# Jittor/JNeRF

Hardware: NVIDIA H100
Metric: ngp_lego_train_rays_per_s (higher is better)
Workload: dtype f16

## Files before the change

### include/ngp_b200.h

```cpp
#ifndef NGP_B200_H
#define NGP_B200_H
#include <stdint.h>
#ifdef __cplusplus
extern "C" {
#endif

#define NGP_F32 0
#define NGP_F16 1
#define NGP_N_LEVELS 16
#define NGP_LEVEL_BYTES 32

const char* ngp_last_error(void);
int ngp_version(void);
int ngp_sm_count(void);
int ngp_debug_timeout_flag(void);

int ngp_hash_offsets(double aabb_scale, int n_levels, int base_resolution, int log2_hashmap_size,
                     uint32_t* offsets_out_host, double* per_level_scale_out);
int ngp_hash_level_table(void* stream, const uint32_t* offsets_host, int n_levels, uint32_t base_resolution,
                         float log2_per_level_scale, void* levels_dev);
int ngp_hash_level_table_primes(void* stream, const uint32_t* offsets_host, int n_levels, uint32_t base_resolution,
                                float log2_per_level_scale, void* levels_dev, uint32_t prime0, uint32_t prime1, uint32_t prime2);

int ngp_hash_fwd(void* stream, uint32_t n, const float* x, const void* grid, int dtype, const void* levels_dev, void* out);
int ngp_hash_bwd(void* stream, uint32_t n, const float* x, const void* dy, int dtype, const void* levels_dev,
                 void* grid_grad, uint64_t n_params);

int ngp_sh_fwd(void* stream, uint32_t n, const float* dirs, int dtype, void* out);

int ngp_mlp_fwd(void* stream, const void* weights, const void* input, void* inter, void* output,
                uint32_t n_hidden_matmuls, uint32_t n);
int ngp_mlp_bwd(void* stream, const void* weights, const void* input, const void* inter, const void* dY,
                void* dX, void* temps, float* dW, uint32_t n_hidden_matmuls, uint32_t n_out_valid, uint32_t n);
int ngp_mlp_bwd_dgrad(void* stream, const void* weights, const void* inter, const void* dY_feature_major, void* dX, void* temps,
                      uint32_t n_hidden_matmuls, uint32_t n);
int ngp_mlp_param_count(uint32_t n_hidden_matmuls);

int ngp_network_fwd(void* stream, uint32_t n_max, const uint32_t* n_dev, const float* coords, const void* grid,
                    const void* levels_dev, const void* w_density, const void* w_rgb, void* out, void* enc_save);
int ngp_network_bwd(void* stream, uint32_t n_max, const uint32_t* n_dev, const float* coords, const void* enc_save,
                    const void* levels_dev, const void* w_density, const void* w_rgb, const void* dout,
                    void* grid_grad, float* dw_density, float* dw_rgb);
int ngp_density_fwd(void* stream, uint32_t n, const float* pos, const void* grid, const void* levels_dev,
                    const void* w_density, void* sigma_out);

int ngp_mesh_workspace_bytes(uint32_t n, uint64_t n_verts, uint64_t n_tris, uint64_t* bytes_out);
int ngp_density_lattice(void* stream, uint32_t n, const void* grid, const void* levels_dev, const void* w_density, float* field_out);
int ngp_marching_cubes(void* stream, uint32_t n, const float* field, float iso, void* workspace, float* verts, uint64_t max_verts,
                       int32_t* tris, uint64_t max_tris, uint64_t* counts_host);
int ngp_mesh_largest_component(void* stream, uint64_t n_verts, uint64_t n_tris, const float* verts, const int32_t* tris, void* workspace,
                               float* verts_out, int32_t* tris_out, uint64_t* counts_host);
int ngp_mesh_vertex_normals(void* stream, uint64_t n_verts, uint64_t n_tris, const float* verts, const int32_t* tris, void* workspace,
                            float* normals);

uint64_t ngp_march_workspace_bytes(uint32_t n_rays);
int ngp_march(void* stream, uint32_t n_rays, float aabb_lo, float aabb_hi, uint32_t max_samples, const float* rays_o,
              const float* rays_d, const uint8_t* bitfield, float cone_angle, float near_distance, uint32_t cascades,
              int const_dt, uint64_t rng_state, uint64_t rng_inc, uint32_t* counters, uint32_t* ray_indices,
              uint32_t* numsteps, float* coords, void* workspace);
int ngp_compact(void* stream, uint32_t n_rays, uint32_t max_compacted, const float* coords_in, const uint32_t* numsteps_in,
                float* coords_out, uint32_t* numsteps_out, uint32_t* counters, int zero_fill);

int ngp_composite_fwd(void* stream, uint32_t n_rays, const void* net_out, int dtype, const float* coords,
                      const uint32_t* numsteps_in, const uint32_t* numsteps_compacted, const float* bg, uint32_t cascades,
                      float* rgb_out);
int ngp_composite_bwd(void* stream, uint32_t n_rays, uint32_t n_elements, const void* net_out, int dtype, const float* coords,
                      const uint32_t* numsteps_compacted, const float* loss_grad, const float* rgb_ray,
                      const float* density_grid_mean, uint32_t cascades, void* dnet_out);
int ngp_composite_infer(void* stream, uint32_t n_rays, const void* net_out, int dtype, const float* coords,
                        const uint32_t* numsteps, uint32_t cascades, float* rgb_out, float* alpha_out);
int ngp_composite_loss_bwd(void* stream, uint32_t n_rays, uint32_t n_elements, const void* net_out, const float* coords,
                           const uint32_t* numsteps_in, const uint32_t* numsteps_compacted, const float* bg,
                           const float* target, float huber_delta, const float* density_grid_mean, uint32_t cascades,
                           float* rgb_out, float* loss_out, void* dnet_out, float reg_scale);

int ngp_render_workspace_bytes(uint32_t n_rays, uint32_t capacity, uint64_t* layout_out);
int ngp_render_init(void* stream, uint32_t n_rays, uint32_t capacity, void* workspace, float aabb_lo, float aabb_hi, const float* rays_o,
                    const float* rays_d, float cone_angle, float near_distance, uint32_t cascades, int const_dt, uint64_t rng_state,
                    uint64_t rng_inc, uint32_t jitter_tile, float* rgb_out, float* alpha_out, uint32_t* n_samples_out, uint32_t* n_alive_host);
int ngp_render_march_round(void* stream, uint32_t n_rays, uint32_t capacity, void* workspace, uint32_t n_alive, uint32_t k_steps, float aabb_lo,
                           float aabb_hi, const float* rays_o, const float* rays_d, const uint8_t* bitfield, float cone_angle, uint32_t cascades,
                           int const_dt);
int ngp_render_composite_round(void* stream, uint32_t n_rays, uint32_t capacity, void* workspace, uint32_t n_alive, uint32_t k_steps,
                               float min_transmittance, uint32_t cascades, float* rgb_out, float* alpha_out, uint32_t* n_samples_out,
                               uint32_t* n_alive_host);

int ngp_grid_mark_untrained(void* stream, uint32_t n_elements, float* grid, uint32_t n_images, const float* focal_lengths,
                            const float* xforms, int res_x, int res_y);
int ngp_grid_generate_samples(void* stream, uint32_t n_elements, uint64_t rng_state, uint64_t rng_inc, const uint32_t* step_dev,
                              float aabb_lo, float aabb_hi, const float* grid_in, float* positions_out, uint32_t* indices_out,
                              uint32_t n_cascades, float thresh);
int ngp_grid_splat(void* stream, uint32_t n, const uint32_t* indices, const void* mlp_out, int dtype, float* grid_tmp);
int ngp_grid_ema(void* stream, uint32_t n_elements, float decay, float* grid, const float* grid_tmp);
int ngp_grid_update_bitfield(void* stream, const float* grid, float* mean_out, uint8_t* bitfield, uint32_t cascades);

int ngp_adam_ema(void* stream, uint64_t n, void* param, int param_dtype, void* grad, int grad_dtype, float grad_scale,
                 float* m, float* v, float* master, float lr, float beta1, float beta2, float eps, uint32_t step,
                 float ema_decay, int zero_grad);

int ngp_dp_exchange_step(void* stream, int world, int rank, uint64_t slice_len, uint32_t n_w, void* const* peer_table,
                         void* const* peer_table_grad, float* const* peer_w_grad, uint32_t* const* peer_flags, uint32_t epoch, float* m,
                         float* v, float* master, void* w_param, float* w_m, float* w_v, float* w_master, float grad_scale, float lr,
                         float beta1, float beta2, float eps, uint32_t step, float ema_decay);
int ngp_dp_exchange_wait(void* stream, int world, const uint32_t* my_flags, uint32_t epoch);
int ngp_ipc_export(const void* dev_ptr, uint8_t* handle64, uint64_t* offset);
int ngp_ipc_open(const uint8_t* handle64, uint64_t offset, void** dev_ptr);
int ngp_ipc_close(void* dev_ptr, uint64_t offset);

int ngp_raygen(void* stream, uint32_t n, const uint32_t* pix_index, uint32_t W, uint32_t H, const float* xforms,
               const float* focal, const float* principal, uint32_t* img_id_out, float* rays_o, float* rays_d);

int ngp_prepare_batch(void* stream, uint32_t n, const uint32_t* pix_index, uint32_t W, uint32_t H, const float* xforms,
                      const float* focal, const float* principal, const void* images_rgba, int image_is_u8, const float* bg,
                      uint32_t* img_id_out, float* rays_o, float* rays_d, float* target);

int ngp_blend_target(void* stream, uint32_t n, const float* rgba, const float* bg, float* target);

uint64_t ngp_step_state_bytes(void);
int ngp_step_state_set(void* stream, void* state_dev, uint64_t rng_state, uint64_t rng_inc, uint32_t pix_cursor, uint32_t adam_steps_done,
                       float lr, float beta1, float beta2, float eps, float ema_decay, float grad_scale);
int ngp_step_state_tick(void* stream, void* state_dev, uint32_t pix_advance, float lr, float beta1, float beta2, float eps,
                        float ema_decay, float grad_scale);
int ngp_prepare_batch_dev(void* stream, uint32_t n, const uint32_t* pix_list, const void* state_dev, uint32_t pix_offset, uint32_t W,
                          uint32_t H, const float* xforms, const float* focal, const float* principal, const void* images_rgba,
                          int image_is_u8, const float* bg, uint32_t* img_id_out, float* rays_o, float* rays_d, float* target);
int ngp_march_dev(void* stream, uint32_t n_rays, float aabb_lo, float aabb_hi, uint32_t max_samples, const float* rays_o,
                  const float* rays_d, const uint8_t* bitfield, float cone_angle, float near_distance, uint32_t cascades, int const_dt,
                  const void* state_dev, uint32_t ray_offset, uint32_t* counters, uint32_t* ray_indices, uint32_t* numsteps,
                  float* coords, void* workspace);
int ngp_adam_ema_dev(void* stream, uint64_t n, void* param, int param_dtype, void* grad, int grad_dtype, float* m, float* v,
                     float* master, const void* state_dev, int zero_grad);

void ngp_pcg32_seed(uint64_t initstate, uint64_t initseq, uint64_t* state_inc);
void ngp_pcg32_advance(uint64_t* state_inc, int64_t delta);

#ifdef __cplusplus
}
#endif
#endif
```

### jnerf_b200/csrc/fused_net.cu

```cuda
#include "mlp_tc.cuh"
#include <cstdlib>
#include <cstdio>
#include <mutex>
#include <vector>

int* ngp_err_flag();

namespace {
using namespace mlp;

constexpr int WD_W0 = 0, WD_WOUT = 64 * 32, WD_N = 64 * 32 + 16 * 64;
constexpr int WR_W0 = 0, WR_W1 = 64 * 32, WR_WOUT = 64 * 32 + 64 * 64, WR_N = 64 * 32 + 64 * 64 + 16 * 64;
constexpr int W_PART = WD_N + WR_N;

constexpr uint32_t G_ENC = 0, G_HD = 4, G_RIN = 12, G_H1 = 16, G_H2F = 4 , G_H2B = 24;
constexpr uint32_t G_ENC1 = 24;
struct SmemFwd {
    static constexpr uint32_t coords = 0;
    static constexpr uint32_t act = 8192;
    static constexpr uint32_t w0d = act + 28 * GB;
    static constexpr uint32_t woutd = w0d + 64 * 32 * 2;
    static constexpr uint32_t w0r = woutd + 16 * 64 * 2;
    static constexpr uint32_t w1r = w0r + 64 * 32 * 2;
    static constexpr uint32_t woutr = w1r + 64 * 64 * 2;
    static constexpr uint32_t levels = woutr + 16 * 64 * 2;
    static constexpr uint32_t total = levels + N_LEVELS * 32;
};
template <class S>
__device__ __forceinline__ void stage_all_weights(uint8_t* smem, const __half* wd, const __half* wr, uint32_t t) {
    stage_weights(smem + S::w0d, wd + WD_W0, 64, 32, t, 128);
    stage_weights(smem + S::woutd, wd + WD_WOUT, 16, 64, t, 128);
    if (wr) {
        stage_weights(smem + S::w0r, wr + WR_W0, 64, 32, t, 128);
        stage_weights(smem + S::w1r, wr + WR_W1, 64, 64, t, 128);
        stage_weights(smem + S::woutr, wr + WR_WOUT, 16, 64, t, 128);
    }
}

template <int STRIDE, int PTS>
__device__ __forceinline__ void gather_tile(const float* __restrict__ s_pos , const NgpLevel& lv,
                                            const __half2* __restrict__ g, uint8_t* act, uint32_t g_enc, uint32_t level, uint32_t sub,
                                            __half* __restrict__ enc_save, uint32_t tile_row0, uint32_t n_live) {
    uint32_t cgx = 0xffffffffu, cgy = 0, cgz = 0;
    __half2 v[8];
#pragma unroll
    for (int c = 0; c < 8; ++c) v[c] = __float2half2_rn(0.f);
#pragma unroll 1
    for (int k = 0; k < PTS; ++k) {
        const uint32_t p = PTS * sub + k;
        const HashCell hc = hash_cell(lv, s_pos[p * STRIDE], s_pos[p * STRIDE + 1], s_pos[p * STRIDE + 2]);
        if (hc.gx != cgx || hc.gy != cgy || hc.gz != cgz) {
            cgx = hc.gx; cgy = hc.gy; cgz = hc.gz;
            uint32_t idx[8];
            hash_cell_indices(lv, cgx, cgy, cgz, idx);
#pragma unroll
            for (int c = 0; c < 8; ++c) v[c] = __ldg(g + idx[c]);
        }
        float w[8];
        hash_cell_weights(hc, w);
        float a0 = 0.f, a1 = 0.f;
#pragma unroll
        for (int c = 0; c < 8; ++c) {
            const float2 f = __half22float2(v[c]);
            a0 = fmaf(w[c], f.x, a0);
            a1 = fmaf(w[c], f.y, a1);
        }
        const __half2 r = __floats2half2_rn(a0, a1);
        *reinterpret_cast<__half2*>(act + (size_t)(g_enc + (level >> 2)) * GB + p * 16 + (level & 3) * 4) = r;
        if (enc_save && tile_row0 + p < n_live)
            *reinterpret_cast<__half2*>(enc_save + (size_t)(tile_row0 + p) * 32 + 2 * level) = r;
    }
}

template <class S, uint32_t G_H2>
__device__ __forceinline__ void forward_chain(uint8_t* smem, uint32_t g_enc , uint32_t tw, bool density_only,
                                              uint32_t bar_id, uint16_t (&sig)[4]) {
    uint8_t* act = smem + S::act;
    const uint32_t smem_s = smem_u32(smem), act_s = smem_s + S::act;
    layer<64>([&](float (&d)[32], uint32_t m) { mma_fwd<32, 64>(d, act_s, g_enc, smem_s + S::w0d, m); },
              [&](const float (&d)[32], uint32_t m) { frag_to_slab<64, true>(d, act, G_HD, m, tw); });
    operands_ready(bar_id, 128);
    layer<16>([&](float (&d)[8], uint32_t m) { mma_fwd<64, 16>(d, act_s, G_HD, smem_s + S::woutd, m); },
              [&](const float (&d)[8], uint32_t m) {
                  sig[2 * m] = (uint16_t)(pack_half2(d[0], d[1]) & 0xFFFFu);
                  sig[2 * m + 1] = (uint16_t)(pack_half2(d[2], d[3]) & 0xFFFFu);
                  if (!density_only) frag_to_slab<16, false>(d, act, G_RIN, m, tw);
              });
    if (density_only) return;
    operands_ready(bar_id, 128);
    layer<64>([&](float (&d)[32], uint32_t m) { mma_fwd<32, 64>(d, act_s, G_RIN, smem_s + S::w0r, m); },
              [&](const float (&d)[32], uint32_t m) { frag_to_slab<64, true>(d, act, G_H1, m, tw); });
    operands_ready(bar_id, 128);
    layer<64>([&](float (&d)[32], uint32_t m) { mma_fwd<64, 64>(d, act_s, G_H1, smem_s + S::w1r, m); },
              [&](const float (&d)[32], uint32_t m) { frag_to_slab<64, true>(d, act, G_H2, m, tw); });
    operands_ready(bar_id, 128);
}
__device__ __forceinline__ void sh_to_slab(uint8_t* act, const float* s_coords, uint32_t t) {
    float sh[16];
    sh4(s_coords[t * 7 + 4], s_coords[t * 7 + 5], s_coords[t * 7 + 6], sh);
    uint32_t p[8];
#pragma unroll
    for (int i = 0; i < 8; ++i) p[i] = pack_half2(sh[2 * i], sh[2 * i + 1]);
    *reinterpret_cast<uint4*>(act + (G_RIN + 2) * GB + t * 16) = make_uint4(p[0], p[1], p[2], p[3]);
    *reinterpret_cast<uint4*>(act + (G_RIN + 3) * GB + t * 16) = make_uint4(p[4], p[5], p[6], p[7]);
}

constexpr int FWD_GW = 8;
constexpr int FWD_THREADS = 128 + 32 * FWD_GW;

__device__ __forceinline__ float lattice_coord(uint32_t r, uint32_t axis, uint32_t n) {
    const uint32_t idx = axis == 0 ? r / (n * n) : axis == 1 ? (r / n) % n : r % n;
    return __fdiv_rn((float)idx, (float)(n - 1));
}

template <bool DENSITY_ONLY, bool LATTICE = false>
__global__ void __launch_bounds__(FWD_THREADS, 2)
network_fwd_kernel(uint32_t n_max, const uint32_t* __restrict__ n_dev, const float* __restrict__ coords, const __half* __restrict__ grid,
                   const NgpLevel* __restrict__ levels, const __half* __restrict__ wd, const __half* __restrict__ wr,
                   __half* __restrict__ out, __half* __restrict__ enc_save, const __grid_constant__ NgpTensorMap enc_map, uint32_t enc_tma,
                   uint32_t lattice_n) {
    static_assert(DENSITY_ONLY || !LATTICE, "the lattice query is density only");
    extern __shared__ __align__(1024) uint8_t smem[];
    using S = SmemFwd;
    constexpr int CS = DENSITY_ONLY ? 3 : 7;
    const uint32_t t = threadIdx.x, warp = t >> 5;
    const bool is_chain = warp < 4;
    NgpLevel* s_lv = reinterpret_cast<NgpLevel*>(smem + S::levels);

    stage_weights(smem + S::w0d, wd + WD_W0, 64, 32, t, FWD_THREADS);
    stage_weights(smem + S::woutd, wd + WD_WOUT, 16, 64, t, FWD_THREADS);
    if (!DENSITY_ONLY) {
        stage_weights(smem + S::w0r, wr + WR_W0, 64, 32, t, FWD_THREADS);
        stage_weights(smem + S::w1r, wr + WR_W1, 64, 64, t, FWD_THREADS);
        stage_weights(smem + S::woutr, wr + WR_WOUT, 16, 64, t, FWD_THREADS);
    }
    if (t < N_LEVELS) s_lv[t] = levels[t];
    operands_ready(0, FWD_THREADS);
    const uint32_t n_live = n_dev ? min(*n_dev, n_max) : n_max;
    const uint32_t ntiles = (n_live + ROWS - 1) / ROWS;

    if (is_chain) {
        uint8_t* act = smem + S::act;
        const uint32_t smem_s = smem_u32(smem), r0 = frag_row(t);
        uint32_t it = 0;
        for (uint32_t tile = blockIdx.x; tile < ntiles; tile += gridDim.x, ++it) {
            const uint32_t buf = it & 1;
            const float* s_coords = reinterpret_cast<const float*>(smem + S::coords + buf * 3584);
            named_bar_sync(2 + buf, FWD_THREADS);
            if (!DENSITY_ONLY && enc_tma && warp == 0) {
                if (elect_one()) {
#pragma unroll
                    for (uint32_t g4 = 0; g4 < 4; ++g4)
                        tma_store_2d(&enc_map, 8 * g4, tile * ROWS, smem_s + S::act + ((buf ? G_ENC1 : G_ENC) + g4) * GB);
                    tma_store_commit();
                }
                __syncwarp();
            }
            if (!DENSITY_ONLY) sh_to_slab(act, s_coords, t);
            uint16_t sig[4];
            forward_chain<S, G_H2F>(smem, buf ? G_ENC1 : G_ENC, t, DENSITY_ONLY, 1, sig);
            if (!DENSITY_ONLY && enc_tma && warp == 0) {
                if (elect_one()) tma_store_wait_read();
                __syncwarp();
            }
            if (tile + 2 * gridDim.x < ntiles) named_bar_arrive(4 + buf, FWD_THREADS);
            if constexpr (DENSITY_ONLY) {
                if ((t & 3u) == 0) {
#pragma unroll
                    for (uint32_t i = 0; i < 4; ++i) {
                        const uint32_t row = tile * ROWS + 64 * (i >> 1) + r0 + 8 * (i & 1);
                        if (row >= n_live) continue;
                        if constexpr (LATTICE) reinterpret_cast<float*>(out)[row] = truncf(fmaxf(__half2float(__ushort_as_half(sig[i])), 0.f));
                        else reinterpret_cast<uint16_t*>(out)[row] = sig[i];
                    }
                }
            } else {
                layer<16>([&](float (&d)[8], uint32_t m) { mma_fwd<64, 16>(d, smem_s + S::act, G_H2F, smem_s + S::woutr, m); },
                          [&](const float (&d)[8], uint32_t m) {
#pragma unroll
                              for (uint32_t h = 0; h < 2; ++h) {
                                  const float c2 = __shfl_down_sync(0xffffffffu, d[2 * h], 1);
                                  const uint32_t row = tile * ROWS + 64 * m + r0 + 8 * h;
                                  if ((t & 3u) == 0 && row < n_live) {
                                      uint2 o;
                                      o.x = pack_half2(d[2 * h], d[2 * h + 1]);
                                      o.y = (pack_half2(c2, 0.f) & 0xFFFFu) | ((uint32_t)sig[2 * m + h] << 16);
                                      reinterpret_cast<uint2*>(out)[row] = o;
                                  }
                              }
                          });
            }
            named_bar_sync(1, 128);
        }
    } else {
        const uint32_t tg = t - 128, level = tg & 15, sub = tg >> 4;
        const NgpLevel lv = s_lv[level];
        const __half2* g = reinterpret_cast<const __half2*>(grid) + lv.offset;
        uint32_t it = 0;
        for (uint32_t tile = blockIdx.x; tile < ntiles; tile += gridDim.x, ++it) {
            const uint32_t buf = it & 1, row0 = tile * ROWS;
            float* s_coords = reinterpret_cast<float*>(smem + S::coords + buf * 3584);
            if (it >= 2) named_bar_sync(4 + buf, FWD_THREADS);
            for (uint32_t i = tg; i < ROWS * CS; i += 32 * FWD_GW) {
                if constexpr (LATTICE) s_coords[i] = (row0 + i / CS < n_live) ? lattice_coord(row0 + i / CS, i % CS, lattice_n) : 0.f;
                else s_coords[i] = (row0 + i / CS < n_live) ? __ldg(coords + (size_t)row0 * CS + i) : 0.f;
            }
            named_bar_sync(6, 32 * FWD_GW);
            gather_tile<CS, 64 / FWD_GW>(s_coords, lv, g, smem + S::act, buf ? G_ENC1 : G_ENC, level, sub, (DENSITY_ONLY || enc_tma) ? nullptr : enc_save, row0,
                                         n_live);
            fence_proxy_async_smem();
            named_bar_arrive(2 + buf, FWD_THREADS);
        }
    }
    if (!DENSITY_ONLY && enc_tma && warp == 0) {
        if (elect_one()) tma_store_wait_all();
        __syncwarp();
    }
}

constexpr uint32_t B3_G_GX = 32, B3_G_DY = 40, B3_G_DENC = 42, B3_GROUPS = 46;
constexpr uint32_t B3_EPI_THREADS = 256, B3_SCATTER_WARPS = 8, B3_THREADS = B3_EPI_THREADS + 32 * B3_SCATTER_WARPS;
constexpr uint32_t B3_RUNS = 12, B3_ITEMS = 16 * B3_RUNS, B3_RUN = (2 * 128 + B3_RUNS - 1) / B3_RUNS;
constexpr uint32_t B3_SCATTER_GROUPS = 32 * B3_SCATTER_WARPS / 4, B3_NI = B3_ITEMS / B3_SCATTER_GROUPS;
static_assert(B3_SCATTER_GROUPS % 16 == 0 && B3_ITEMS % B3_SCATTER_GROUPS == 0, "a lane group walks items of one level only, as many as every other group");
struct SmemBwd3 {
    static constexpr uint32_t coords = 0;
    static constexpr uint32_t tile0 = coords + 4 * 3584;
    static constexpr uint32_t tile_stride = B3_GROUPS * GB;
    static constexpr uint32_t w0d = tile0 + 2 * tile_stride;
    static constexpr uint32_t woutd = w0d + 64 * 32 * 2;
    static constexpr uint32_t w0r = woutd + 16 * 64 * 2;
    static constexpr uint32_t w1r = w0r + 64 * 32 * 2;
    static constexpr uint32_t woutr = w1r + 64 * 64 * 2;
    static constexpr uint32_t levels = woutr + 16 * 64 * 2;
    static constexpr uint32_t dsig = levels + N_LEVELS * 32;
    static constexpr uint32_t bar = dsig + 2 * ROWS * 2;
    static constexpr uint32_t total = bar + 16;
};
static_assert(SmemBwd3::total <= 227 * 1024, "backward CTA does not fit");
constexpr uint32_t B3_STAGE = 1, B3_FULL = 2, B3_EMPTY = 3;

constexpr float FX_SCALE = 4294967296.0f, FX_INV = 1.0f / 4294967296.0f;
__device__ __forceinline__ void red_add_fx(unsigned long long* p, float v) {
    const long long q = __float2ll_rn(fminf(fmaxf(v, -65504.f), 65504.f) * FX_SCALE);
    if (q) asm volatile("red.global.add.u64 [%0], %1;" ::"l"(__cvta_generic_to_global(p)), "l"((unsigned long long)q) : "memory");
}
__device__ __forceinline__ void red_add_entry_lane(unsigned long long* fx, uint32_t fx_live, __half2* gg, uint32_t idx, uint32_t f, float v) {
    if (idx < fx_live) {
        red_add_fx(fx + 2 * (size_t)idx + f, v);
    } else {
        const uint32_t lane = threadIdx.x & 31;
        const float o = __shfl_xor_sync(3u << (lane & 30), v, 1);
        if (!f) red_add_h2(gg + idx, v, o);
    }
}

template <uint32_t T>
__device__ __forceinline__ void bwd_chain(uint8_t* smem, uint32_t tid, uint32_t n_live, uint32_t npairs, const float* __restrict__ coords,
                                          const __half* __restrict__ enc_save, const __half* __restrict__ dout, float* __restrict__ w_part,
                                          float* __restrict__ dwd, float* __restrict__ dwr, int* __restrict__ err, uint32_t dbg, const NgpTensorMap* enc_map, uint32_t enc_tma) {
    using S = SmemBwd3;
    const uint32_t t = tid & 127, tq = (tid >> 5) & 3, r0 = frag_row(t);
    uint8_t* act = smem + S::tile0 + T * S::tile_stride;
    const uint32_t smem_s = smem_u32(smem), a0 = smem_s + S::tile0, a1 = a0 + S::tile_stride, a_s = T ? a1 : a0;
    __half* s_dsig = reinterpret_cast<__half*>(smem + S::dsig) + T * ROWS;
    uint64_t* bar_t = reinterpret_cast<uint64_t*>(smem + S::bar) + T;
    const bool wg = !(dbg & 4);
    float acc_woutr[8] = {}, acc_w1r[32] = {};
    float acc_w0r[16] = {}, acc_woutd[8] = {}, acc_w0d[16] = {};
    auto stage = [&]() { operands_ready(B3_STAGE, B3_EPI_THREADS); };
    float pf_c[7];
    uint4 pf_e[4];
    uint2 pf_d;
    auto prefetch = [&](uint32_t pair) {
        const uint32_t tile_ = 2 * pair + T, rr0 = tile_ * ROWS, r = rr0 + t;
        const bool ok = r < n_live;
#pragma unroll
        for (int j = 0; j < 7; ++j) {
            const uint32_t i = t + 128 * j;
            pf_c[j] = (rr0 + i / 7 < n_live) ? __ldg(coords + (size_t)rr0 * 7 + i) : 0.f;
        }
        if (!enc_tma) {
            const uint4* es = reinterpret_cast<const uint4*>(enc_save + (size_t)r * 32);
#pragma unroll
            for (int g = 0; g < 4; ++g) pf_e[g] = ok ? __ldg(es + g) : make_uint4(0, 0, 0, 0);
        }
        pf_d = ok ? __ldg(reinterpret_cast<const uint2*>(dout) + r) : make_uint2(0, 0);
    };
    if (blockIdx.x < npairs) prefetch(blockIdx.x);
    uint32_t it = 0, acc = 0;
    for (uint32_t pair = blockIdx.x; pair < npairs; pair += gridDim.x, ++it, acc = 1) {
        const uint32_t buf = it & 1;
        float* s_coords = reinterpret_cast<float*>(smem + S::coords + (2 * T + buf) * 3584);
        if (it >= 1) named_bar_sync(B3_STAGE, B3_EPI_THREADS);
#pragma unroll
        for (int j = 0; j < 7; ++j) s_coords[t + 128 * j] = pf_c[j];
        if (enc_tma) {
            if (tq == 0) {
                if (elect_one()) {
                    mbar_expect_tx(bar_t, ROWS * 64);
#pragma unroll
                    for (uint32_t g4 = 0; g4 < 4; ++g4)
                        tma_load_2d(smem_u32(act) + (G_ENC + g4) * GB, enc_map, 8 * g4, (2 * pair + T) * ROWS, bar_t);
                }
                __syncwarp();
            }
        } else {
#pragma unroll
            for (int g = 0; g < 4; ++g) *reinterpret_cast<uint4*>(act + (G_ENC + g) * GB + t * 16) = pf_e[g];
        }
        s_dsig[t] = __ushort_as_half((unsigned short)(pf_d.y >> 16));
        *reinterpret_cast<uint4*>(act + B3_G_DY * GB + t * 16) = make_uint4(pf_d.x, pf_d.y & 0xFFFFu, 0, 0);
        *reinterpret_cast<uint4*>(act + (B3_G_DY + 1) * GB + t * 16) = make_uint4(0, 0, 0, 0);
        if (pair + gridDim.x < npairs) prefetch(pair + gridDim.x);
        if (enc_tma) {
            if (!mbar_wait(bar_t, it & 1)) atomicExch(err, 4);
            if ((2 * pair + T) * ROWS + t >= n_live) {
#pragma unroll
                for (int g = 0; g < 4; ++g) *reinterpret_cast<uint4*>(act + (G_ENC + g) * GB + t * 16) = make_uint4(0, 0, 0, 0);
            }
        }
        named_bar_sync(4 + T, 128);
        sh_to_slab(act, s_coords, t);
        stage();
        layer<64>([&](float (&d)[32], uint32_t m) { mma_fwd<32, 64>(d, a_s, G_ENC, smem_s + S::w0d, m); },
                  [&](const float (&d)[32], uint32_t m) { frag_to_slab<64, true>(d, act, G_HD, m, t); });
        stage();
        layer<16>([&](float (&d)[8], uint32_t m) { mma_fwd<64, 16>(d, a_s, G_HD, smem_s + S::woutd, m); },
                  [&](const float (&d)[8], uint32_t m) { frag_to_slab<16, false>(d, act, G_RIN, m, t); });
        stage();
        layer<64>([&](float (&d)[32], uint32_t m) { mma_fwd<32, 64>(d, a_s, G_RIN, smem_s + S::w0r, m); },
                  [&](const float (&d)[32], uint32_t m) { frag_to_slab<64, true>(d, act, G_H1, m, t); });
        stage();
        layer<64>([&](float (&d)[32], uint32_t m) { mma_fwd<64, 64>(d, a_s, G_H1, smem_s + S::w1r, m); },
                  [&](const float (&d)[32], uint32_t m) { frag_to_slab<64, true>(d, act, G_H2B, m, t); });
        stage();
        if (T == 0 && wg) { wgmma_fence(); mma_wgrad<16>(acc_woutr, a0, G_H2B, a0, B3_G_DY, acc); mma_wgrad<16>(acc_woutr, a1, G_H2B, a1, B3_G_DY, 1); }
        layer<64>([&](float (&d)[32], uint32_t m) { mma_dgrad<16, 64>(d, a_s, B3_G_DY, smem_s + S::woutr, m); },
                  [&](const float (&d)[32], uint32_t m) { frag_dgrad_mask<64>(d, act, G_H2B, act, B3_G_GX, m, t); });
        stage();
        if (T == 0 && wg) { wgmma_fence(); mma_wgrad<64>(acc_w1r, a0, B3_G_GX, a0, G_H1, acc); mma_wgrad<64>(acc_w1r, a1, B3_G_GX, a1, G_H1, 1); }
        layer<64>([&](float (&d)[32], uint32_t m) { mma_dgrad<64, 64>(d, a_s, B3_G_GX, smem_s + S::w1r, m); },
                  [&](const float (&d)[32], uint32_t m) { frag_dgrad_mask<64>(d, act, G_H1, act, G_H2B, m, t); });
        stage();
        if (T == 1 && wg) { wgmma_fence(); mma_wgrad<32>(acc_w0r, a0, G_H2B, a0, G_RIN, acc); mma_wgrad<32>(acc_w0r, a1, G_H2B, a1, G_RIN, 1); }
        layer<16>([&](float (&d)[8], uint32_t m) { mma_dgrad<64, 16>(d, a_s, G_H2B, smem_s + S::w0r, m); },
                  [&](const float (&d)[8], uint32_t m) {
                      float v[8];
#pragma unroll
                      for (int i = 0; i < 8; ++i) v[i] = d[i];
                      if ((t & 3u) == 0) {
                          v[0] += __half2float(s_dsig[64 * m + r0]);
                          v[2] += __half2float(s_dsig[64 * m + r0 + 8]);
                      }
                      frag_to_slab<16, false>(v, act, B3_G_DY, m, t);
                  });
        stage();
        if (T == 1 && wg) { wgmma_fence(); mma_wgrad<16>(acc_woutd, a0, G_HD, a0, B3_G_DY, acc); mma_wgrad<16>(acc_woutd, a1, G_HD, a1, B3_G_DY, 1); }
        layer<64>([&](float (&d)[32], uint32_t m) { mma_dgrad<16, 64>(d, a_s, B3_G_DY, smem_s + S::woutd, m); },
                  [&](const float (&d)[32], uint32_t m) { frag_dgrad_mask<64>(d, act, G_HD, act, G_H1, m, t); });
        stage();
        if (T == 1 && wg) { wgmma_fence(); mma_wgrad<32>(acc_w0d, a0, G_H1, a0, G_ENC, acc); mma_wgrad<32>(acc_w0d, a1, G_H1, a1, G_ENC, 1); }
        if (it >= 1) named_bar_sync(B3_EMPTY, B3_EPI_THREADS + 32 * B3_SCATTER_WARPS);
        layer<32>([&](float (&d)[16], uint32_t m) { mma_dgrad<64, 32>(d, a_s, G_H1, smem_s + S::w0d, m); },
                  [&](const float (&d)[16], uint32_t m) { frag_to_slab<32, false>(d, act, B3_G_DENC, m, t); });
        named_bar_arrive(B3_FULL, B3_EPI_THREADS + 32 * B3_SCATTER_WARPS);
    }
    if (!w_part) {
        if (!it) return;
        if (T == 0) {
            frag_red_add<16>(acc_woutr, dwr + WR_WOUT, 1, 64, 64, 3, t);
            frag_red_add<64>(acc_w1r, dwr + WR_W1, 64, 1, 64, 64, t);
        } else {
            frag_red_add<32>(acc_w0r, dwr + WR_W0, 32, 1, 64, 32, t);
            frag_red_add<16>(acc_woutd, dwd + WD_WOUT, 1, 64, 64, 16, t);
            frag_red_add<32>(acc_w0d, dwd + WD_W0, 32, 1, 64, 32, t);
        }
        return;
    }
    dwd = w_part + (size_t)blockIdx.x * W_PART;
    dwr = dwd + WD_N;
    if (T == 0) {
        frag_store<16>(acc_woutr, dwr + WR_WOUT, 1, 64, 3, t);
        frag_store<64>(acc_w1r, dwr + WR_W1, 64, 1, 64, t);
    } else {
        frag_store<32>(acc_w0r, dwr + WR_W0, 32, 1, 32, t);
        frag_store<16>(acc_woutd, dwd + WD_WOUT, 1, 64, 16, t);
        frag_store<32>(acc_w0d, dwd + WD_W0, 32, 1, 32, t);
    }
}

__global__ void __launch_bounds__(B3_THREADS, 1)
network_bwd256_kernel(uint32_t n_max, const uint32_t* __restrict__ n_dev, const float* __restrict__ coords, const __half* __restrict__ enc_save,
                      const NgpLevel* __restrict__ levels, const __half* __restrict__ wd, const __half* __restrict__ wr,
                      const __half* __restrict__ dout, __half* __restrict__ grid_grad, float* __restrict__ dwd, float* __restrict__ dwr,
                      unsigned long long* __restrict__ grid_fx, uint32_t fx_entries, float* __restrict__ w_part,
                      int* __restrict__ err, uint32_t dbg, const __grid_constant__ NgpTensorMap enc_map, uint32_t enc_tma) {
    extern __shared__ __align__(1024) uint8_t smem[];
    using S = SmemBwd3;
    const uint32_t tid = threadIdx.x, warp = tid >> 5;
    uint64_t* bar_t = reinterpret_cast<uint64_t*>(smem + S::bar);
    NgpLevel* s_lv = reinterpret_cast<NgpLevel*>(smem + S::levels);

    stage_weights(smem + S::w0d, wd + WD_W0, 64, 32, tid, B3_THREADS);
    stage_weights(smem + S::woutd, wd + WD_WOUT, 16, 64, tid, B3_THREADS);
    stage_weights(smem + S::w0r, wr + WR_W0, 64, 32, tid, B3_THREADS);
    stage_weights(smem + S::w1r, wr + WR_W1, 64, 64, tid, B3_THREADS);
    stage_weights(smem + S::woutr, wr + WR_WOUT, 16, 64, tid, B3_THREADS);
    if (tid < N_LEVELS) s_lv[tid] = levels[tid];
    for (uint32_t i = tid; i < 2 * S::tile_stride / 16; i += B3_THREADS) *reinterpret_cast<uint4*>(smem + S::tile0 + i * 16) = make_uint4(0, 0, 0, 0);
    if (tid == 0) { mbar_init(bar_t, 1); mbar_init(bar_t + 1, 1); fence_mbar_init(); }
    operands_ready(0, B3_THREADS);
    const uint32_t n_live = n_dev ? min(*n_dev, n_max) : n_max;
    const uint32_t ntiles = (n_live + ROWS - 1) / ROWS, npairs = (ntiles + 1) / 2;

    if (warp < 4) {
        bwd_chain<0>(smem, tid, n_live, npairs, coords, enc_save, dout, w_part, dwd, dwr, err, dbg, &enc_map, enc_tma);
    } else if (warp < 8) {
        bwd_chain<1>(smem, tid, n_live, npairs, coords, enc_save, dout, w_part, dwd, dwr, err, dbg, &enc_map, enc_tma);
    } else {
        const uint32_t ts = tid - B3_EPI_THREADS, grp = ts >> 2, f = ts & 1, h = (ts >> 1) & 1;
        const uint32_t level = grp & 15;
        const NgpLevel lv = s_lv[level];
        unsigned long long* fx = grid_fx + 2 * (size_t)lv.offset;
        const uint32_t fx_live = fx_entries > lv.offset ? fx_entries - lv.offset : 0u;
        __half2* gg = reinterpret_cast<__half2*>(grid_grad) + lv.offset;
        uint32_t it = 0;
        for (uint32_t pair = blockIdx.x; pair < npairs; pair += gridDim.x, ++it) {
            const uint32_t buf = it & 1;
            named_bar_sync(B3_FULL, B3_EPI_THREADS + 32 * B3_SCATTER_WARPS);
            uint32_t cgx[B3_NI], cgy[B3_NI], cgz[B3_NI], idx[B3_NI][4];
            float acc[B3_NI][4];
            bool live[B3_NI], dirty[B3_NI];
#pragma unroll
            for (uint32_t i = 0; i < B3_NI; ++i) { cgx[i] = 0xffffffffu; cgy[i] = cgz[i] = 0; live[i] = !(dbg & 2); dirty[i] = false; }
#pragma unroll 1
            for (uint32_t k = 0; k < B3_RUN; ++k) {
                float2 df[B3_NI];
                HashCell hc[B3_NI];
#pragma unroll
                for (uint32_t i = 0; i < B3_NI; ++i) {
                    const uint32_t r = B3_RUN * ((grp + i * B3_SCATTER_GROUPS) >> 4) + k;
                    live[i] = live[i] && r < 2 * ROWS && 2 * pair * ROWS + r < n_live;
                    const uint32_t rc = min(r, 2 * ROWS - 1), T = rc >> 7, p = rc & 127;
                    const uint8_t* denc = smem + S::tile0 + T * S::tile_stride + B3_G_DENC * GB;
                    const float* s_coords = reinterpret_cast<const float*>(smem + S::coords + (2 * T + buf) * 3584);
                    df[i] = __half22float2(*reinterpret_cast<const __half2*>(denc + (size_t)(level >> 2) * GB + p * 16 + (level & 3) * 4));
                    hc[i] = hash_cell(lv, s_coords[p * 7], s_coords[p * 7 + 1], s_coords[p * 7 + 2]);
                }
#pragma unroll
                for (uint32_t i = 0; i < B3_NI; ++i) {
                    if (!live[i] || (df[i].x == 0.f && df[i].y == 0.f)) continue;
                    if (hc[i].gx != cgx[i] || hc[i].gy != cgy[i] || hc[i].gz != cgz[i]) {
                        if (dirty[i] && !(dbg & 1)) {
#pragma unroll
                            for (uint32_t j = 0; j < 4; ++j) red_add_entry_lane(fx, fx_live, gg, idx[i][j], f, acc[i][j]);
                        }
                        cgx[i] = hc[i].gx; cgy[i] = hc[i].gy; cgz[i] = hc[i].gz;
                        uint32_t ci[8];
                        hash_cell_indices(lv, cgx[i], cgy[i], cgz[i], ci);
#pragma unroll
                        for (uint32_t j = 0; j < 4; ++j) { idx[i][j] = h ? ci[2 * j + 1] : ci[2 * j]; acc[i][j] = 0.f; }
                        dirty[i] = true;
                    }
                    const float dv = f ? df[i].y : df[i].x;
                    const float wx = h ? hc[i].fx : 1.0f - hc[i].fx;
                    const float wy[2] = {1.0f - hc[i].fy, hc[i].fy}, wz[2] = {1.0f - hc[i].fz, hc[i].fz};
#pragma unroll
                    for (uint32_t j = 0; j < 4; ++j) acc[i][j] = fmaf(dv, (1.0f * wx) * wy[j & 1] * wz[j >> 1], acc[i][j]);
                }
            }
#pragma unroll
            for (uint32_t i = 0; i < B3_NI; ++i) {
                if (dirty[i] && !(dbg & 1)) {
#pragma unroll
                    for (uint32_t j = 0; j < 4; ++j) red_add_entry_lane(fx, fx_live, gg, idx[i][j], f, acc[i][j]);
                }
            }
            if (pair + gridDim.x < npairs) named_bar_arrive(B3_EMPTY, B3_EPI_THREADS + 32 * B3_SCATTER_WARPS);
        }
    }
}

__global__ void wgrad_reduce_kernel(const float* __restrict__ part, uint32_t nparts, float* __restrict__ dwd, float* __restrict__ dwr) {
    const uint32_t e = blockIdx.x * blockDim.x + threadIdx.x;
    if (e >= (uint32_t)W_PART) return;
    float a0 = 0.f, a1 = 0.f, a2 = 0.f, a3 = 0.f;
    uint32_t k = 0;
#pragma unroll 4
    for (; k + 4 <= nparts; k += 4) {
        a0 += part[(size_t)k * W_PART + e];
        a1 += part[(size_t)(k + 1) * W_PART + e];
        a2 += part[(size_t)(k + 2) * W_PART + e];
        a3 += part[(size_t)(k + 3) * W_PART + e];
    }
    for (; k < nparts; ++k) a0 += part[(size_t)k * W_PART + e];
    const float sum = (a0 + a1) + (a2 + a3);
    if (e < (uint32_t)WD_N) dwd[e] += sum; else dwr[e - WD_N] += sum;
}

__global__ void grid_grad_flush_kernel(const NgpLevel* __restrict__ levels, uint32_t fx_entries, longlong2* __restrict__ fx,
                                       __half2* __restrict__ grid_grad) {
    const uint32_t n = min(levels[N_LEVELS - 1].offset + levels[N_LEVELS - 1].size, fx_entries);
    for (uint32_t i = blockIdx.x * blockDim.x + threadIdx.x; i < n; i += gridDim.x * blockDim.x) {
        const longlong2 q = fx[i];
        if (q.x | q.y) {
            float2 g = __half22float2(grid_grad[i]);
            g.x += __ll2float_rn(q.x) * FX_INV;
            g.y += __ll2float_rn(q.y) * FX_INV;
            grid_grad[i] = __floats2half2_rn(g.x, g.y);
            fx[i] = make_longlong2(0, 0);
        }
    }
}

struct BwdScratch {
    int dev = -1;
    cudaStream_t stream = nullptr;
    const void* levels = nullptr;
    uint32_t fx_entries = 0;
    unsigned long long* fx = nullptr;
    float* part = nullptr;
};
std::mutex g_scratch_mu;
std::vector<BwdScratch*> g_scratch;

int bwd_scratch(cudaStream_t s, const void* levels_dev, BwdScratch** out) {
    *out = nullptr;
    int dev = 0;
    NGP_CHECK_CUDA(cudaGetDevice(&dev));
    BwdScratch* b = nullptr;
    {
        std::lock_guard<std::mutex> lock(g_scratch_mu);
        for (BwdScratch* e : g_scratch)
            if (e->dev == dev && e->stream == s) b = e;
        if (!b) {
            b = new BwdScratch;
            b->dev = dev;
            b->stream = s;
            g_scratch.push_back(b);
        }
    }
    if (b->levels == levels_dev && b->part) { *out = b; return 0; }
    cudaStreamCaptureStatus cap = cudaStreamCaptureStatusNone;
    NGP_CHECK_CUDA(cudaStreamIsCapturing(s, &cap));
    if (cap != cudaStreamCaptureStatusNone) return 0;
    NgpLevel last;
    NGP_CHECK_CUDA(cudaMemcpyAsync(&last, reinterpret_cast<const NgpLevel*>(levels_dev) + N_LEVELS - 1, sizeof(last), cudaMemcpyDeviceToHost, s));
    NGP_CHECK_CUDA(cudaStreamSynchronize(s));
    const uint32_t entries = last.offset + last.size;
    if (entries > b->fx_entries) {
        if (b->fx) NGP_CHECK_CUDA(cudaFree(b->fx));
        b->fx = nullptr;
        b->fx_entries = 0;
        NGP_CHECK_CUDA(cudaMalloc(&b->fx, sizeof(unsigned long long) * 2 * (size_t)entries));
        NGP_CHECK_CUDA(cudaMemset(b->fx, 0, sizeof(unsigned long long) * 2 * (size_t)entries));
        b->fx_entries = entries;
    }
    if (!b->part) NGP_CHECK_CUDA(cudaMalloc(&b->part, sizeof(float) * W_PART * (size_t)ngp_num_sms()));
    b->levels = levels_dev;
    *out = b;
    return 0;
}

}

extern "C" {

int ngp_network_fwd(void* stream, uint32_t n_max, const uint32_t* n_dev, const float* coords, const void* grid, const void* levels_dev,
                    const void* w_density, const void* w_rgb, void* out, void* enc_save) {
    if (n_max == 0) return 0;
    cudaStream_t s = (cudaStream_t)stream;
    if (ngp_first_use((const void*)network_fwd_kernel<false>)) NGP_CHECK_CUDA(cudaFuncSetAttribute(network_fwd_kernel<false>, cudaFuncAttributeMaxDynamicSharedMemorySize, (int)SmemFwd::total));
    const uint32_t ntiles = (n_max + ROWS - 1) / ROWS;
    const uint32_t grid_dim = min(ntiles, (uint32_t)ngp_num_sms() * 2u);
    NgpTensorMap enc_map{};
    static const bool no_tma = getenv("NGP_NO_TMA") != nullptr;
    const uint32_t enc_tma = (!no_tma && enc_save && ngp_make_rows32_tensormap(&enc_map, enc_save, n_max)) ? 1u : 0u;
    network_fwd_kernel<false><<<grid_dim, FWD_THREADS, SmemFwd::total, s>>>(n_max, n_dev, coords, (const __half*)grid, (const NgpLevel*)levels_dev,
                                                                   (const __half*)w_density, (const __half*)w_rgb, (__half*)out,
                                                                   (__half*)enc_save, enc_map, enc_tma, 0u);
    NGP_LAUNCH_CHECK();
    return 0;
}

int ngp_density_fwd(void* stream, uint32_t n, const float* pos, const void* grid, const void* levels_dev, const void* w_density, void* sigma_out) {
    if (n == 0) return 0;
    cudaStream_t s = (cudaStream_t)stream;
    if (ngp_first_use((const void*)network_fwd_kernel<true>)) NGP_CHECK_CUDA(cudaFuncSetAttribute(network_fwd_kernel<true>, cudaFuncAttributeMaxDynamicSharedMemorySize, (int)SmemFwd::total));
    const uint32_t ntiles = (n + ROWS - 1) / ROWS;
    const uint32_t grid_dim = min(ntiles, (uint32_t)ngp_num_sms() * 2u);
    network_fwd_kernel<true><<<grid_dim, FWD_THREADS, SmemFwd::total, s>>>(n, nullptr, pos, (const __half*)grid, (const NgpLevel*)levels_dev,
                                                                  (const __half*)w_density, nullptr, (__half*)sigma_out, nullptr, NgpTensorMap{}, 0u, 0u);
    NGP_LAUNCH_CHECK();
    return 0;
}

int ngp_density_lattice(void* stream, uint32_t n, const void* grid, const void* levels_dev, const void* w_density, float* field_out) {
    NGP_REQUIRE(n >= 2 && n <= 1024, "ngp_density_lattice: resolution n must be in [2, 1024], got " + std::to_string(n));
    cudaStream_t s = (cudaStream_t)stream;
    if (ngp_first_use((const void*)network_fwd_kernel<true, true>))
        NGP_CHECK_CUDA(cudaFuncSetAttribute(network_fwd_kernel<true, true>, cudaFuncAttributeMaxDynamicSharedMemorySize, (int)SmemFwd::total));
    const uint32_t n3 = n * n * n, ntiles = (n3 + ROWS - 1) / ROWS;
    const uint32_t grid_dim = min(ntiles, (uint32_t)ngp_num_sms() * 2u);
    network_fwd_kernel<true, true><<<grid_dim, FWD_THREADS, SmemFwd::total, s>>>(n3, nullptr, nullptr, (const __half*)grid, (const NgpLevel*)levels_dev,
                                                                                (const __half*)w_density, nullptr, reinterpret_cast<__half*>(field_out),
                                                                                nullptr, NgpTensorMap{}, 0u, n);
    NGP_LAUNCH_CHECK();
    return 0;
}

int ngp_network_bwd(void* stream, uint32_t n_max, const uint32_t* n_dev, const float* coords, const void* enc_save, const void* levels_dev,
                    const void* w_density, const void* w_rgb, const void* dout, void* grid_grad, float* dw_density, float* dw_rgb) {
    if (n_max == 0) return 0;
    cudaStream_t s = (cudaStream_t)stream;
    const uint32_t ntiles = (n_max + ROWS - 1) / ROWS;
    static const uint32_t dbg = getenv("NGP_BWD_DEBUG") ? (uint32_t)atoi(getenv("NGP_BWD_DEBUG")) : 0u;
    if (ngp_first_use((const void*)network_bwd256_kernel)) NGP_CHECK_CUDA(cudaFuncSetAttribute(network_bwd256_kernel, cudaFuncAttributeMaxDynamicSharedMemorySize, (int)SmemBwd3::total));
    const uint32_t grid_dim = min((ntiles + 1) / 2, (uint32_t)ngp_num_sms());
    NgpTensorMap enc_map{};
    static const bool no_tma = getenv("NGP_NO_TMA") != nullptr;
    const uint32_t enc_tma = (!no_tma && ngp_make_rows32_tensormap(&enc_map, enc_save, n_max)) ? 1u : 0u;
    BwdScratch* b = nullptr;
    if (int rc = bwd_scratch(s, levels_dev, &b)) return rc;
    network_bwd256_kernel<<<grid_dim, B3_THREADS, SmemBwd3::total, s>>>(n_max, n_dev, coords, (const __half*)enc_save, (const NgpLevel*)levels_dev,
                                                                       (const __half*)w_density, (const __half*)w_rgb, (const __half*)dout,
                                                                       (__half*)grid_grad, dw_density, dw_rgb, b ? b->fx : nullptr,
                                                                       b ? b->fx_entries : 0u, b ? b->part : nullptr, ngp_err_flag(), dbg, enc_map, enc_tma);
    NGP_LAUNCH_CHECK();
    if (b) {
        wgrad_reduce_kernel<<<(W_PART + 255) / 256, 256, 0, s>>>(b->part, grid_dim, dw_density, dw_rgb);
        NGP_LAUNCH_CHECK();
        grid_grad_flush_kernel<<<ngp_num_sms() * 8, 256, 0, s>>>((const NgpLevel*)levels_dev, b->fx_entries, reinterpret_cast<longlong2*>(b->fx),
                                                                 (__half2*)grid_grad);
        NGP_LAUNCH_CHECK();
    }
    return 0;
}

}
```

### jnerf_b200/csrc/optimizer.cu

```cuda
#include "ngp_common.cuh"
#include <cmath>
#include <cstring>

namespace {

__device__ __forceinline__ float adam_one(float g, float& m, float& v, float& master, const AdamArgs& a) {
    g = __fmul_rn(g, a.grad_scale);
    m = __fmaf_rn(a.b1, m, __fmul_rn(1.f - a.b1, g));
    v = __fmaf_rn(a.b2, v, __fmul_rn(__fmul_rn(1.f - a.b2, g), g));
    const float p = __fsub_rn(master, __fdiv_rn(__fmul_rn(m, a.step_size), __fadd_rn(sqrtf(v), a.eps)));
    master = __fmul_rn(__fmaf_rn(1.f - a.decay, p, __fmul_rn(__fmul_rn(a.decay, master), a.debias_old)), a.debias_new);
    return master;
}

template <typename PT, typename GT>
__global__ void __launch_bounds__(256) adam_ema_kernel(uint64_t n, PT* __restrict__ param, GT* __restrict__ grad, float* __restrict__ m,
                                                       float* __restrict__ v, float* __restrict__ master, AdamArgs a, int zero_grad,
                                                       const NgpStepState* __restrict__ st) {
    if (st) a = st->adam;
    constexpr int UNROLL = 2;
    const uint64_t n4 = n / 4, T = (uint64_t)gridDim.x * blockDim.x, g = blockIdx.x * (uint64_t)blockDim.x + threadIdx.x;
    for (uint64_t i0 = g; i0 < n4; i0 += UNROLL * T) {
        float4 gr[UNROLL], mm[UNROLL], vv[UNROLL], ms[UNROLL];
#pragma unroll
        for (int u = 0; u < UNROLL; ++u) {
            const uint64_t i = i0 + u * T;
            if (i < n4) {
                if constexpr (sizeof(GT) == 2) {
                    const uint2 w = reinterpret_cast<const uint2*>(grad)[i];
                    const float2 f0 = __half22float2(*reinterpret_cast<const __half2*>(&w.x)), f1 = __half22float2(*reinterpret_cast<const __half2*>(&w.y));
                    gr[u] = make_float4(f0.x, f0.y, f1.x, f1.y);
                } else {
                    gr[u] = reinterpret_cast<const float4*>(grad)[i];
                }
                mm[u] = reinterpret_cast<const float4*>(m)[i];
                vv[u] = reinterpret_cast<const float4*>(v)[i];
                ms[u] = reinterpret_cast<const float4*>(master)[i];
            }
        }
#pragma unroll
        for (int u = 0; u < UNROLL; ++u) {
            const uint64_t i = i0 + u * T;
            if (i < n4) {
                float4 p;
                p.x = adam_one(gr[u].x, mm[u].x, vv[u].x, ms[u].x, a);
                p.y = adam_one(gr[u].y, mm[u].y, vv[u].y, ms[u].y, a);
                p.z = adam_one(gr[u].z, mm[u].z, vv[u].z, ms[u].z, a);
                p.w = adam_one(gr[u].w, mm[u].w, vv[u].w, ms[u].w, a);
                reinterpret_cast<float4*>(m)[i] = mm[u];
                reinterpret_cast<float4*>(v)[i] = vv[u];
                reinterpret_cast<float4*>(master)[i] = ms[u];
                if constexpr (sizeof(PT) == 2) {
                    __half2 h0 = __floats2half2_rn(p.x, p.y), h1 = __floats2half2_rn(p.z, p.w);
                    uint2 o;
                    o.x = *reinterpret_cast<uint32_t*>(&h0);
                    o.y = *reinterpret_cast<uint32_t*>(&h1);
                    reinterpret_cast<uint2*>(param)[i] = o;
                } else {
                    reinterpret_cast<float4*>(param)[i] = p;
                }
                if (zero_grad) {
                    if constexpr (sizeof(GT) == 2) reinterpret_cast<uint2*>(grad)[i] = make_uint2(0, 0);
                    else reinterpret_cast<float4*>(grad)[i] = make_float4(0, 0, 0, 0);
                }
            }
        }
    }
    if (blockIdx.x == 0 && threadIdx.x < (n & 3)) {
        const uint64_t i = n4 * 4 + threadIdx.x;
        float g1 = (float)grad[i], m1 = m[i], v1 = v[i], s1 = master[i];
        if (zero_grad) grad[i] = (GT)0.f;
        const float p = adam_one(g1, m1, v1, s1, a);
        m[i] = m1; v[i] = v1; master[i] = s1; param[i] = (PT)p;
    }
}

__global__ void raygen_kernel(uint32_t n, const uint32_t* __restrict__ pix, uint32_t W, uint32_t H, const float* __restrict__ xforms,
                              const float* __restrict__ focal, const float* __restrict__ principal, uint32_t* __restrict__ img_id,
                              float* __restrict__ rays_o, float* __restrict__ rays_d) {
    const uint32_t i = blockIdx.x * blockDim.x + threadIdx.x;
    if (i >= n) return;
    const uint32_t id = pix[i] / (H * W), off = pix[i] % (H * W);
    const float* m = xforms + 12 * (size_t)id;
    const float x = ((off % W) + 0.5f) / W, y = ((off / W) + 0.5f) / H;
    const float dx = (x - principal[2 * id]) * W / focal[2 * id], dy = (y - principal[2 * id + 1]) * H / focal[2 * id + 1];
    const float d0 = m[0] * dx + m[3] * dy + m[6], d1 = m[1] * dx + m[4] * dy + m[7], d2 = m[2] * dx + m[5] * dy + m[8];
    const float nrm = fmaxf(sqrtf(d0 * d0 + d1 * d1 + d2 * d2), 1e-12f);
    img_id[i] = id;
    rays_o[3 * (size_t)i] = m[9]; rays_o[3 * (size_t)i + 1] = m[10]; rays_o[3 * (size_t)i + 2] = m[11];
    rays_d[3 * (size_t)i] = d0 / nrm; rays_d[3 * (size_t)i + 1] = d1 / nrm; rays_d[3 * (size_t)i + 2] = d2 / nrm;
}

template <typename IMG>
__global__ void prepare_batch_kernel(uint32_t n, const uint32_t* __restrict__ pix, uint32_t W, uint32_t H, const float* __restrict__ xforms,
                                     const float* __restrict__ focal, const float* __restrict__ principal, const IMG* __restrict__ images,
                                     const float* __restrict__ bg, uint32_t* __restrict__ img_id, float* __restrict__ rays_o,
                                     float* __restrict__ rays_d, float* __restrict__ target, const NgpStepState* __restrict__ st,
                                     uint32_t pix_offset) {
    const uint32_t i = blockIdx.x * blockDim.x + threadIdx.x;
    if (i >= n) return;
    const uint32_t px = pix[(st ? st->pix_cursor : 0u) + pix_offset + i];
    const uint32_t id = px / (H * W), off = px % (H * W);
    const float* m = xforms + 12 * (size_t)id;
    const float x = ((off % W) + 0.5f) / W, y = ((off / W) + 0.5f) / H;
    const float dx = (x - principal[2 * id]) * W / focal[2 * id], dy = (y - principal[2 * id + 1]) * H / focal[2 * id + 1];
    const float d0 = m[0] * dx + m[3] * dy + m[6], d1 = m[1] * dx + m[4] * dy + m[7], d2 = m[2] * dx + m[5] * dy + m[8];
    const float nrm = fmaxf(sqrtf(d0 * d0 + d1 * d1 + d2 * d2), 1e-12f);
    img_id[i] = id;
    rays_o[3 * (size_t)i] = m[9]; rays_o[3 * (size_t)i + 1] = m[10]; rays_o[3 * (size_t)i + 2] = m[11];
    rays_d[3 * (size_t)i] = d0 / nrm; rays_d[3 * (size_t)i + 1] = d1 / nrm; rays_d[3 * (size_t)i + 2] = d2 / nrm;
    float4 c;
    if constexpr (sizeof(IMG) == 1) {
        const uchar4 u = reinterpret_cast<const uchar4*>(images)[px];
        c = make_float4(u.x / 255.0f, u.y / 255.0f, u.z / 255.0f, u.w / 255.0f);
    } else {
        c = reinterpret_cast<const float4*>(images)[px];
    }
    const float ia = 1.0f - c.w;
    target[3 * (size_t)i] = c.x * c.w + bg[3 * (size_t)i] * ia;
    target[3 * (size_t)i + 1] = c.y * c.w + bg[3 * (size_t)i + 1] * ia;
    target[3 * (size_t)i + 2] = c.z * c.w + bg[3 * (size_t)i + 2] * ia;
}

__global__ void blend_target_kernel(uint32_t n, const float4* __restrict__ rgba, const float* __restrict__ bg, float* __restrict__ target) {
    const uint32_t i = blockIdx.x * blockDim.x + threadIdx.x;
    if (i >= n) return;
    const float4 c = rgba[i];
    const float ia = 1.0f - c.w;
    target[3 * (size_t)i] = c.x * c.w + bg[3 * (size_t)i] * ia;
    target[3 * (size_t)i + 1] = c.y * c.w + bg[3 * (size_t)i + 1] * ia;
    target[3 * (size_t)i + 2] = c.z * c.w + bg[3 * (size_t)i + 2] * ia;
}

constexpr int DP_MAX_WORLD = 16;
constexpr int DP_FLAG_GRADS = 0, DP_FLAG_DONE = 16, DP_FLAG_COUNTER = 32, DP_FLAG_WORDS = 64;

struct DpPeers {
    __half* table[DP_MAX_WORLD];
    __half* table_grad[DP_MAX_WORLD];
    float* w_grad[DP_MAX_WORLD];
    uint32_t* flags[DP_MAX_WORLD];
};

__device__ __forceinline__ void st_release_sys(uint32_t* p, uint32_t v) {
    asm volatile("st.release.sys.global.u32 [%0], %1;" ::"l"(p), "r"(v) : "memory");
}
__device__ __forceinline__ uint32_t ld_acquire_sys(const uint32_t* p) {
    uint32_t v;
    asm volatile("ld.acquire.sys.global.u32 %0, [%1];" : "=r"(v) : "l"(p) : "memory");
    return v;
}
__device__ __forceinline__ uint64_t global_timer_ns() {
    uint64_t t;
    asm volatile("mov.u64 %0, %%globaltimer;" : "=l"(t));
    return t;
}
__device__ __forceinline__ void wait_flag(const uint32_t* p, uint32_t epoch) {
    const uint64_t t0 = global_timer_ns();
#pragma unroll 1
    while ((int32_t)(ld_acquire_sys(p) - epoch) < 0) {
        if (global_timer_ns() - t0 > 20ull * 1000000000ull) __trap();
    }
}

__global__ void __launch_bounds__(256, 2) dp_exchange_kernel(DpPeers P, int W, int rank, uint64_t slice_len, uint32_t n_w, uint32_t epoch,
                                                          float* m, float* v, float* master, __half* w_param, float* w_m, float* w_v,
                                                          float* w_master, AdamArgs a) {
    if (blockIdx.x == 0 && threadIdx.x < W) {
        __threadfence_system();
        st_release_sys(P.flags[threadIdx.x] + DP_FLAG_GRADS + rank, epoch);
    }
    if (threadIdx.x < W) wait_flag(P.flags[rank] + DP_FLAG_GRADS + threadIdx.x, epoch);
    __syncthreads();

    const uint64_t lo = (uint64_t)rank * slice_len, n8 = slice_len / 8;
    const uint64_t T = (uint64_t)gridDim.x * blockDim.x;
    for (uint64_t i = blockIdx.x * (uint64_t)blockDim.x + threadIdx.x; i < n8; i += T) {
        float g[8] = {0.f, 0.f, 0.f, 0.f, 0.f, 0.f, 0.f, 0.f};
        uint4 w[DP_MAX_WORLD];
#pragma unroll
        for (int r = 0; r < DP_MAX_WORLD; ++r)
            if (r < W) w[r] = *reinterpret_cast<uint4*>(P.table_grad[r] + lo + 8 * i);
        float4 mm[2], vv[2], ms[2];
#pragma unroll
        for (int h = 0; h < 2; ++h) {
            mm[h] = reinterpret_cast<const float4*>(m)[2 * i + h];
            vv[h] = reinterpret_cast<const float4*>(v)[2 * i + h];
            ms[h] = reinterpret_cast<const float4*>(master)[2 * i + h];
        }
#pragma unroll
        for (int r = 0; r < DP_MAX_WORLD; ++r) {
            if (r < W) {
                const uint32_t u[4] = {w[r].x, w[r].y, w[r].z, w[r].w};
#pragma unroll
                for (int k = 0; k < 4; ++k) {
                    const float2 f = __half22float2(*reinterpret_cast<const __half2*>(&u[k]));
                    g[2 * k] += f.x;
                    g[2 * k + 1] += f.y;
                }
            }
        }
        float p[8];
#pragma unroll
        for (int h = 0; h < 2; ++h) {
            p[4 * h + 0] = adam_one(g[4 * h + 0], mm[h].x, vv[h].x, ms[h].x, a);
            p[4 * h + 1] = adam_one(g[4 * h + 1], mm[h].y, vv[h].y, ms[h].y, a);
            p[4 * h + 2] = adam_one(g[4 * h + 2], mm[h].z, vv[h].z, ms[h].z, a);
            p[4 * h + 3] = adam_one(g[4 * h + 3], mm[h].w, vv[h].w, ms[h].w, a);
            reinterpret_cast<float4*>(m)[2 * i + h] = mm[h];
            reinterpret_cast<float4*>(v)[2 * i + h] = vv[h];
            reinterpret_cast<float4*>(master)[2 * i + h] = ms[h];
        }
        uint4 o;
        {
            __half2 h0 = __floats2half2_rn(p[0], p[1]), h1 = __floats2half2_rn(p[2], p[3]), h2 = __floats2half2_rn(p[4], p[5]),
                    h3 = __floats2half2_rn(p[6], p[7]);
            o.x = *reinterpret_cast<uint32_t*>(&h0);
            o.y = *reinterpret_cast<uint32_t*>(&h1);
            o.z = *reinterpret_cast<uint32_t*>(&h2);
            o.w = *reinterpret_cast<uint32_t*>(&h3);
        }
#pragma unroll
        for (int r = 0; r < DP_MAX_WORLD; ++r)
            if (r < W) *reinterpret_cast<uint4*>(P.table[r] + lo + 8 * i) = o;
    }
    for (uint32_t j = blockIdx.x * blockDim.x + threadIdx.x; j < n_w; j += (uint32_t)T) {
        float g = 0.f;
        for (int r = 0; r < W; ++r) g += P.w_grad[r][j];
        float m1 = w_m[j], v1 = w_v[j], s1 = w_master[j];
        const float p = adam_one(g, m1, v1, s1, a);
        w_m[j] = m1; w_v[j] = v1; w_master[j] = s1;
        w_param[j] = __float2half_rn(p);
    }
    __threadfence_system();
    __syncthreads();
    __shared__ bool last;
    uint32_t* mine = P.flags[rank];
    if (threadIdx.x == 0) last = atomicAdd(mine + DP_FLAG_COUNTER, 1u) == gridDim.x - 1;
    __syncthreads();
    if (last) {
        __threadfence();
        if (threadIdx.x < W) st_release_sys(P.flags[threadIdx.x] + DP_FLAG_DONE + rank, epoch);
        if (threadIdx.x == 0) mine[DP_FLAG_COUNTER] = 0;
    }
}

__global__ void dp_wait_kernel(const uint32_t* my_flags, int W, uint32_t epoch) {
    if (threadIdx.x < W) wait_flag(my_flags + DP_FLAG_DONE + threadIdx.x, epoch);
}

}

extern "C" {

static AdamArgs make_adam_args(float lr, float beta1, float beta2, float eps, uint32_t step, float ema_decay, float grad_scale);

static int adam_launch(void* stream, uint64_t n, void* param, int param_dtype, void* grad, int grad_dtype, float* m, float* v, float* master,
                       AdamArgs a, int zero_grad, const NgpStepState* st) {
    if (n == 0) return 0;
    cudaStream_t s = (cudaStream_t)stream;
    const uint64_t n4 = (n + 3) / 4;
    const uint32_t blocks = (uint32_t)std::max<uint64_t>(1, std::min<uint64_t>((n4 + 511) / 512, (uint64_t)ngp_num_sms() * 32));
    if (param_dtype == 1 && grad_dtype == 1) adam_ema_kernel<__half, __half><<<blocks, 256, 0, s>>>(n, (__half*)param, (__half*)grad, m, v, master, a, zero_grad, st);
    else if (param_dtype == 1 && grad_dtype == 0) adam_ema_kernel<__half, float><<<blocks, 256, 0, s>>>(n, (__half*)param, (float*)grad, m, v, master, a, zero_grad, st);
    else if (param_dtype == 0 && grad_dtype == 0) adam_ema_kernel<float, float><<<blocks, 256, 0, s>>>(n, (float*)param, (float*)grad, m, v, master, a, zero_grad, st);
    else NGP_REQUIRE(false, "ngp_adam_ema: unsupported dtype combination");
    NGP_LAUNCH_CHECK();
    return 0;
}

int ngp_adam_ema(void* stream, uint64_t n, void* param, int param_dtype, void* grad, int grad_dtype, float grad_scale, float* m, float* v,
                 float* master, float lr, float beta1, float beta2, float eps, uint32_t step, float ema_decay, int zero_grad) {
    NGP_REQUIRE(step >= 1, "ngp_adam_ema: step is 1-based");
    return adam_launch(stream, n, param, param_dtype, grad, grad_dtype, m, v, master, make_adam_args(lr, beta1, beta2, eps, step, ema_decay, grad_scale),
                       zero_grad, nullptr);
}

int ngp_adam_ema_dev(void* stream, uint64_t n, void* param, int param_dtype, void* grad, int grad_dtype, float* m, float* v, float* master,
                     const void* state_dev, int zero_grad) {
    NGP_REQUIRE(state_dev != nullptr, "ngp_adam_ema_dev: state_dev is required");
    return adam_launch(stream, n, param, param_dtype, grad, grad_dtype, m, v, master, AdamArgs{}, zero_grad, (const NgpStepState*)state_dev);
}

static AdamArgs make_adam_args(float lr, float beta1, float beta2, float eps, uint32_t step, float ema_decay, float grad_scale) {
    AdamArgs a;
    const double n1 = 1.0 - std::pow((double)beta1, (double)step), n2 = 1.0 - std::pow((double)beta2, (double)step);
    a.step_size = (float)(lr * std::sqrt(n2) / n1);
    a.b1 = beta1; a.b2 = beta2; a.eps = eps; a.decay = ema_decay; a.grad_scale = grad_scale;
    a.debias_old = (float)(1.0 - std::pow((double)ema_decay, (double)step - 1.0));
    a.debias_new = (float)(1.0 / (1.0 - std::pow((double)ema_decay, (double)step)));
    return a;
}

int ngp_dp_exchange_step(void* stream, int world, int rank, uint64_t slice_len, uint32_t n_w, void* const* peer_table,
                         void* const* peer_table_grad, float* const* peer_w_grad, uint32_t* const* peer_flags, uint32_t epoch, float* m,
                         float* v, float* master, void* w_param, float* w_m, float* w_v, float* w_master, float grad_scale, float lr,
                         float beta1, float beta2, float eps, uint32_t step, float ema_decay) {
    NGP_REQUIRE(world >= 1 && world <= DP_MAX_WORLD && rank >= 0 && rank < world, "ngp_dp_exchange_step: world must be 1..16 and rank < world");
    NGP_REQUIRE(slice_len % 256 == 0, "ngp_dp_exchange_step: slice_len must be a multiple of 256 (dp.padded_len)");
    NGP_REQUIRE(step >= 1 && epoch >= 1, "ngp_dp_exchange_step: step and epoch are 1-based");
    DpPeers P;
    for (int r = 0; r < DP_MAX_WORLD; ++r) {
        const int q = r < world ? r : rank;
        P.table[r] = (__half*)peer_table[q];
        P.table_grad[r] = (__half*)peer_table_grad[q];
        P.w_grad[r] = peer_w_grad[q];
        P.flags[r] = peer_flags[q];
    }
    const AdamArgs a = make_adam_args(lr, beta1, beta2, eps, step, ema_decay, grad_scale);
    const uint64_t n8 = slice_len / 8;
    const uint32_t blocks = (uint32_t)std::max<uint64_t>(1, std::min<uint64_t>((n8 + 255) / 256, (uint64_t)ngp_num_sms() * 2));
    dp_exchange_kernel<<<blocks, 256, 0, (cudaStream_t)stream>>>(P, world, rank, slice_len, n_w, epoch, m, v, master, (__half*)w_param, w_m, w_v,
                                                                 w_master, a);
    NGP_LAUNCH_CHECK();
    return 0;
}

int ngp_dp_exchange_wait(void* stream, int world, const uint32_t* my_flags, uint32_t epoch) {
    NGP_REQUIRE(world >= 1 && world <= DP_MAX_WORLD, "ngp_dp_exchange_wait: world must be 1..16");
    dp_wait_kernel<<<1, 32, 0, (cudaStream_t)stream>>>(my_flags, world, epoch);
    NGP_LAUNCH_CHECK();
    return 0;
}

int ngp_ipc_export(const void* dev_ptr, uint8_t* handle64, uint64_t* offset) {
    typedef int (*GetRange)(unsigned long long*, size_t*, unsigned long long);
    void* fn = nullptr;
    cudaDriverEntryPointQueryResult qr;
    NGP_CHECK_CUDA(cudaGetDriverEntryPoint("cuMemGetAddressRange", &fn, cudaEnableDefault, &qr));
    NGP_REQUIRE(fn != nullptr && qr == cudaDriverEntryPointSuccess, "ngp_ipc_export: cuMemGetAddressRange not available");
    unsigned long long base = 0;
    size_t size = 0;
    NGP_REQUIRE(((GetRange)fn)(&base, &size, (unsigned long long)(uintptr_t)dev_ptr) == 0, "ngp_ipc_export: not a device allocation");
    cudaIpcMemHandle_t h;
    NGP_CHECK_CUDA(cudaIpcGetMemHandle(&h, (void*)(uintptr_t)base));
    static_assert(sizeof(h) == 64, "cudaIpcMemHandle_t is 64 bytes");
    memcpy(handle64, &h, 64);
    *offset = (uint64_t)((uintptr_t)dev_ptr - (uintptr_t)base);
    return 0;
}

int ngp_ipc_open(const uint8_t* handle64, uint64_t offset, void** dev_ptr) {
    cudaIpcMemHandle_t h;
    memcpy(&h, handle64, 64);
    void* base = nullptr;
    NGP_CHECK_CUDA(cudaIpcOpenMemHandle(&base, h, cudaIpcMemLazyEnablePeerAccess));
    *dev_ptr = (void*)((uintptr_t)base + offset);
    return 0;
}

int ngp_ipc_close(void* dev_ptr, uint64_t offset) {
    NGP_CHECK_CUDA(cudaIpcCloseMemHandle((void*)((uintptr_t)dev_ptr - offset)));
    return 0;
}

static int prepare_batch_launch(void* stream, uint32_t n, const uint32_t* pix, uint32_t W, uint32_t H, const float* xforms, const float* focal,
                                const float* principal, const void* images_rgba, int image_is_u8, const float* bg, uint32_t* img_id_out,
                                float* rays_o, float* rays_d, float* target, const NgpStepState* st, uint32_t pix_offset) {
    if (n == 0) return 0;
    cudaStream_t s = (cudaStream_t)stream;
    if (image_is_u8) prepare_batch_kernel<uint8_t><<<(n + 127) / 128, 128, 0, s>>>(n, pix, W, H, xforms, focal, principal, (const uint8_t*)images_rgba, bg, img_id_out, rays_o, rays_d, target, st, pix_offset);
    else prepare_batch_kernel<float><<<(n + 127) / 128, 128, 0, s>>>(n, pix, W, H, xforms, focal, principal, (const float*)images_rgba, bg, img_id_out, rays_o, rays_d, target, st, pix_offset);
    NGP_LAUNCH_CHECK();
    return 0;
}

int ngp_prepare_batch(void* stream, uint32_t n, const uint32_t* pix_index, uint32_t W, uint32_t H, const float* xforms, const float* focal,
                      const float* principal, const void* images_rgba, int image_is_u8, const float* bg, uint32_t* img_id_out, float* rays_o,
                      float* rays_d, float* target) {
    return prepare_batch_launch(stream, n, pix_index, W, H, xforms, focal, principal, images_rgba, image_is_u8, bg, img_id_out, rays_o, rays_d, target,
                                nullptr, 0);
}

int ngp_prepare_batch_dev(void* stream, uint32_t n, const uint32_t* pix_list, const void* state_dev, uint32_t pix_offset, uint32_t W, uint32_t H,
                          const float* xforms, const float* focal, const float* principal, const void* images_rgba, int image_is_u8,
                          const float* bg, uint32_t* img_id_out, float* rays_o, float* rays_d, float* target) {
    NGP_REQUIRE(state_dev != nullptr, "ngp_prepare_batch_dev: state_dev is required");
    return prepare_batch_launch(stream, n, pix_list, W, H, xforms, focal, principal, images_rgba, image_is_u8, bg, img_id_out, rays_o, rays_d, target,
                                (const NgpStepState*)state_dev, pix_offset);
}

__global__ void step_state_set_kernel(NgpStepState* st, uint64_t rng_state, uint64_t rng_inc, uint32_t pix_cursor, uint32_t steps_done, AdamArgs next) {
    st->rng_state = rng_state; st->rng_inc = rng_inc; st->pix_cursor = pix_cursor; st->adam_steps_done = steps_done; st->adam = next;
}
__global__ void step_state_tick_kernel(NgpStepState* st, uint32_t pix_advance, float lr, float beta1, float beta2, float eps, float ema_decay,
                                       float grad_scale) {
    Pcg32 rng{st->rng_state, st->rng_inc};
    rng.advance((int64_t)1 << 32);
    st->rng_state = rng.state;
    st->pix_cursor += pix_advance;
    const uint32_t done = st->adam_steps_done + 1;
    st->adam_steps_done = done;
    const double step = (double)done + 1.0;
    const double n1 = 1.0 - pow((double)beta1, step), n2 = 1.0 - pow((double)beta2, step);
    AdamArgs a;
    a.step_size = (float)((double)lr * sqrt(n2) / n1);
    a.b1 = beta1; a.b2 = beta2; a.eps = eps; a.decay = ema_decay; a.grad_scale = grad_scale;
    a.debias_old = (float)(1.0 - pow((double)ema_decay, step - 1.0));
    a.debias_new = (float)(1.0 / (1.0 - pow((double)ema_decay, step)));
    st->adam = a;
}

uint64_t ngp_step_state_bytes(void) { return sizeof(NgpStepState); }

int ngp_step_state_set(void* stream, void* state_dev, uint64_t rng_state, uint64_t rng_inc, uint32_t pix_cursor, uint32_t adam_steps_done, float lr,
                       float beta1, float beta2, float eps, float ema_decay, float grad_scale) {
    step_state_set_kernel<<<1, 1, 0, (cudaStream_t)stream>>>((NgpStepState*)state_dev, rng_state, rng_inc, pix_cursor, adam_steps_done,
                                                              make_adam_args(lr, beta1, beta2, eps, adam_steps_done + 1, ema_decay, grad_scale));
    NGP_LAUNCH_CHECK();
    return 0;
}

int ngp_step_state_tick(void* stream, void* state_dev, uint32_t pix_advance, float lr, float beta1, float beta2, float eps, float ema_decay,
                        float grad_scale) {
    step_state_tick_kernel<<<1, 1, 0, (cudaStream_t)stream>>>((NgpStepState*)state_dev, pix_advance, lr, beta1, beta2, eps, ema_decay, grad_scale);
    NGP_LAUNCH_CHECK();
    return 0;
}

int ngp_blend_target(void* stream, uint32_t n, const float* rgba, const float* bg, float* target) {
    if (n == 0) return 0;
    blend_target_kernel<<<(n + 127) / 128, 128, 0, (cudaStream_t)stream>>>(n, reinterpret_cast<const float4*>(rgba), bg, target);
    NGP_LAUNCH_CHECK();
    return 0;
}

int ngp_raygen(void* stream, uint32_t n, const uint32_t* pix_index, uint32_t W, uint32_t H, const float* xforms, const float* focal,
               const float* principal, uint32_t* img_id_out, float* rays_o, float* rays_d) {
    if (n == 0) return 0;
    raygen_kernel<<<(n + 127) / 128, 128, 0, (cudaStream_t)stream>>>(n, pix_index, W, H, xforms, focal, principal, img_id_out, rays_o, rays_d);
    NGP_LAUNCH_CHECK();
    return 0;
}

}
```

### jnerf_b200/lib.py

```python
import ctypes as C
import os

HERE = os.path.dirname(os.path.abspath(__file__))
LIB_PATH = os.environ.get("NGP_B200_LIB") or os.path.join(HERE, "libngp_b200.so")

_vp, _u32, _u64, _i64, _f32, _i32, _f64 = C.c_void_p, C.c_uint32, C.c_uint64, C.c_int64, C.c_float, C.c_int, C.c_double

SIGNATURES = {
    "ngp_last_error": (C.c_char_p, []),
    "ngp_version": (_i32, []),
    "ngp_sm_count": (_i32, []),
    "ngp_debug_timeout_flag": (_i32, []),
    "ngp_hash_offsets": (_i32, [_f64, _i32, _i32, _i32, _vp, _vp]),
    "ngp_hash_level_table": (_i32, [_vp, _vp, _i32, _u32, _f32, _vp]),
    "ngp_hash_level_table_primes": (_i32, [_vp, _vp, _i32, _u32, _f32, _vp, _u32, _u32, _u32]),
    "ngp_hash_fwd": (_i32, [_vp, _u32, _vp, _vp, _i32, _vp, _vp]),
    "ngp_hash_bwd": (_i32, [_vp, _u32, _vp, _vp, _i32, _vp, _vp, _u64]),
    "ngp_sh_fwd": (_i32, [_vp, _u32, _vp, _i32, _vp]),
    "ngp_mlp_fwd": (_i32, [_vp, _vp, _vp, _vp, _vp, _u32, _u32]),
    "ngp_mlp_bwd": (_i32, [_vp, _vp, _vp, _vp, _vp, _vp, _vp, _vp, _u32, _u32, _u32]),
    "ngp_mlp_bwd_dgrad": (_i32, [_vp, _vp, _vp, _vp, _vp, _vp, _u32, _u32]),
    "ngp_mlp_param_count": (_i32, [_u32]),
    "ngp_network_fwd": (_i32, [_vp, _u32, _vp, _vp, _vp, _vp, _vp, _vp, _vp, _vp]),
    "ngp_network_bwd": (_i32, [_vp, _u32, _vp, _vp, _vp, _vp, _vp, _vp, _vp, _vp, _vp, _vp]),
    "ngp_density_fwd": (_i32, [_vp, _u32, _vp, _vp, _vp, _vp, _vp]),
    "ngp_mesh_workspace_bytes": (_i32, [_u32, _u64, _u64, _vp]),
    "ngp_density_lattice": (_i32, [_vp, _u32, _vp, _vp, _vp, _vp]),
    "ngp_marching_cubes": (_i32, [_vp, _u32, _vp, _f32, _vp, _vp, _u64, _vp, _u64, _vp]),
    "ngp_mesh_largest_component": (_i32, [_vp, _u64, _u64, _vp, _vp, _vp, _vp, _vp, _vp]),
    "ngp_mesh_vertex_normals": (_i32, [_vp, _u64, _u64, _vp, _vp, _vp, _vp]),
    "ngp_render_workspace_bytes": (_i32, [_u32, _u32, _vp]),
    "ngp_render_init": (_i32, [_vp, _u32, _u32, _vp, _f32, _f32, _vp, _vp, _f32, _f32, _u32, _i32, _u64, _u64, _u32, _vp, _vp, _vp, _vp]),
    "ngp_render_march_round": (_i32, [_vp, _u32, _u32, _vp, _u32, _u32, _f32, _f32, _vp, _vp, _vp, _f32, _u32, _i32]),
    "ngp_render_composite_round": (_i32, [_vp, _u32, _u32, _vp, _u32, _u32, _f32, _u32, _vp, _vp, _vp, _vp]),
    "ngp_march_workspace_bytes": (_u64, [_u32]),
    "ngp_march": (_i32, [_vp, _u32, _f32, _f32, _u32, _vp, _vp, _vp, _f32, _f32, _u32, _i32, _u64, _u64, _vp, _vp, _vp, _vp, _vp]),
    "ngp_compact": (_i32, [_vp, _u32, _u32, _vp, _vp, _vp, _vp, _vp, _i32]),
    "ngp_composite_fwd": (_i32, [_vp, _u32, _vp, _i32, _vp, _vp, _vp, _vp, _u32, _vp]),
    "ngp_composite_bwd": (_i32, [_vp, _u32, _u32, _vp, _i32, _vp, _vp, _vp, _vp, _vp, _u32, _vp]),
    "ngp_composite_infer": (_i32, [_vp, _u32, _vp, _i32, _vp, _vp, _u32, _vp, _vp]),
    "ngp_composite_loss_bwd": (_i32, [_vp, _u32, _u32, _vp, _vp, _vp, _vp, _vp, _vp, _f32, _vp, _u32, _vp, _vp, _vp, _f32]),
    "ngp_grid_mark_untrained": (_i32, [_vp, _u32, _vp, _u32, _vp, _vp, _i32, _i32]),
    "ngp_grid_generate_samples": (_i32, [_vp, _u32, _u64, _u64, _vp, _f32, _f32, _vp, _vp, _vp, _u32, _f32]),
    "ngp_grid_splat": (_i32, [_vp, _u32, _vp, _vp, _i32, _vp]),
    "ngp_grid_ema": (_i32, [_vp, _u32, _f32, _vp, _vp]),
    "ngp_grid_update_bitfield": (_i32, [_vp, _vp, _vp, _vp, _u32]),
    "ngp_adam_ema": (_i32, [_vp, _u64, _vp, _i32, _vp, _i32, _f32, _vp, _vp, _vp, _f32, _f32, _f32, _f32, _u32, _f32, _i32]),
    "ngp_dp_exchange_step": (_i32, [_vp, _i32, _i32, _u64, _u32, _vp, _vp, _vp, _vp, _u32, _vp, _vp, _vp, _vp, _vp, _vp, _vp, _f32, _f32, _f32,
                                    _f32, _f32, _u32, _f32]),
    "ngp_dp_exchange_wait": (_i32, [_vp, _i32, _vp, _u32]),
    "ngp_ipc_export": (_i32, [_vp, _vp, _vp]),
    "ngp_ipc_open": (_i32, [_vp, _u64, _vp]),
    "ngp_ipc_close": (_i32, [_vp, _u64]),
    "ngp_raygen": (_i32, [_vp, _u32, _vp, _u32, _u32, _vp, _vp, _vp, _vp, _vp, _vp]),
    "ngp_prepare_batch": (_i32, [_vp, _u32, _vp, _u32, _u32, _vp, _vp, _vp, _vp, _i32, _vp, _vp, _vp, _vp, _vp]),
    "ngp_blend_target": (_i32, [_vp, _u32, _vp, _vp, _vp]),
    "ngp_step_state_bytes": (_u64, []),
    "ngp_step_state_set": (_i32, [_vp, _vp, _u64, _u64, _u32, _u32, _f32, _f32, _f32, _f32, _f32, _f32]),
    "ngp_step_state_tick": (_i32, [_vp, _vp, _u32, _f32, _f32, _f32, _f32, _f32, _f32]),
    "ngp_prepare_batch_dev": (_i32, [_vp, _u32, _vp, _vp, _u32, _u32, _u32, _vp, _vp, _vp, _vp, _i32, _vp, _vp, _vp, _vp, _vp]),
    "ngp_march_dev": (_i32, [_vp, _u32, _f32, _f32, _u32, _vp, _vp, _vp, _f32, _f32, _u32, _i32, _vp, _u32, _vp, _vp, _vp, _vp, _vp]),
    "ngp_adam_ema_dev": (_i32, [_vp, _u64, _vp, _i32, _vp, _i32, _vp, _vp, _vp, _vp, _i32]),
    "ngp_pcg32_seed": (None, [_u64, _u64, _vp]),
    "ngp_pcg32_advance": (None, [_vp, _i64]),
}

KERNELS_PER_CALL = {
    "ngp_hash_level_table": 1, "ngp_hash_level_table_primes": 1, "ngp_hash_fwd": 1, "ngp_hash_bwd": 1, "ngp_sh_fwd": 1, "ngp_mlp_fwd": 1, "ngp_mlp_bwd": 1, "ngp_mlp_bwd_dgrad": 1,
    "ngp_network_fwd": 1, "ngp_network_bwd": 1, "ngp_density_fwd": 1, "ngp_march": 3, "ngp_compact": 1, "ngp_composite_fwd": 1,
    "ngp_composite_bwd": 1, "ngp_composite_infer": 1, "ngp_composite_loss_bwd": 1, "ngp_grid_mark_untrained": 1,
    "ngp_grid_generate_samples": 1, "ngp_grid_splat": 1, "ngp_grid_ema": 1, "ngp_grid_update_bitfield": 7, "ngp_adam_ema": 1, "ngp_dp_exchange_step": 1, "ngp_dp_exchange_wait": 1, "ngp_raygen": 1, "ngp_prepare_batch": 1,
    "ngp_blend_target": 1, "ngp_step_state_set": 1, "ngp_step_state_tick": 1, "ngp_prepare_batch_dev": 1, "ngp_march_dev": 3, "ngp_adam_ema_dev": 1,
    "ngp_density_lattice": 1, "ngp_marching_cubes": 3, "ngp_mesh_largest_component": 18, "ngp_mesh_vertex_normals": 7,
    "ngp_render_init": 3, "ngp_render_march_round": 3, "ngp_render_composite_round": 3,
}
launch_count = 0
_lib = None


class NgpError(RuntimeError):
    pass


def load():
    global _lib
    if _lib is None:
        if not os.path.exists(LIB_PATH):
            raise NgpError(f"{LIB_PATH} is missing: build it with `python jnerf_b200/build.py` (nvcc, sm_90a). "
                           "There is no CPU fallback.")
        lib = C.CDLL(LIB_PATH)
        for name, (res, args) in SIGNATURES.items():
            fn = getattr(lib, name)
            fn.restype = res
            fn.argtypes = args
        _lib = lib
    return _lib


def call(name, *args):
    global launch_count
    lib = load()
    launch_count += KERNELS_PER_CALL.get(name, 0)
    rc = getattr(lib, name)(*args)
    if rc != 0:
        raise NgpError(f"{name} failed ({rc}): {lib.ngp_last_error().decode()}")
    return rc
```

### jnerf_b200/ops.py

```python
import numpy as np
import torch

from . import lib

F32, F16 = 0, 1


def _dt(t):
    if t.dtype == torch.float16:
        return F16
    if t.dtype == torch.float32:
        return F32
    raise TypeError(f"unsupported dtype {t.dtype}")


def _p(t):
    if t is None:
        return None
    assert t.is_cuda and t.is_contiguous(), "device-resident contiguous tensor required"
    return t.data_ptr()


_raw_stream, _raw_device = getattr(torch._C, "_cuda_getCurrentRawStream", None), getattr(torch._C, "_cuda_getDevice", None)


def _stream():
    if _raw_stream is not None and _raw_device is not None:
        return _raw_stream(_raw_device())
    return torch.cuda.current_stream().cuda_stream


class HashLevels:

    def __init__(self, aabb_scale=1, n_levels=16, base_resolution=16, log2_hashmap_size=19, device="cuda", primes=(1, 19349663, 83492791)):
        import ctypes as C
        self.primes = tuple(int(p) & 0xFFFFFFFF for p in primes)
        self.n_levels, self.base_resolution = n_levels, base_resolution
        self.offsets = np.zeros(n_levels + 1, np.uint32)
        pls = C.c_double()
        lib.call("ngp_hash_offsets", float(aabb_scale), n_levels, base_resolution, log2_hashmap_size, self.offsets.ctypes.data, C.addressof(pls))
        self.per_level_scale = pls.value
        self.log2_per_level_scale = float(np.float32(np.log2(self.per_level_scale)))
        self.n_entries = int(self.offsets[-1])
        self.n_params = 2 * self.n_entries
        self.table = torch.empty(n_levels * 32, dtype=torch.uint8, device=device)
        lib.call("ngp_hash_level_table_primes", _stream(), self.offsets.ctypes.data, n_levels, base_resolution, self.log2_per_level_scale,
                 _p(self.table), *self.primes)


def hash_fwd(x, grid, levels):
    out = torch.empty((x.shape[0], 32), dtype=grid.dtype, device=x.device)
    lib.call("ngp_hash_fwd", _stream(), x.shape[0], _p(x), _p(grid), _dt(grid), _p(levels.table), _p(out))
    return out


def hash_bwd(x, dy, levels, grid_grad=None):
    if grid_grad is None:
        alloc = torch.zeros if x.shape[0] == 0 else torch.empty
        grid_grad = alloc(levels.n_params, dtype=dy.dtype, device=x.device)
    lib.call("ngp_hash_bwd", _stream(), x.shape[0], _p(x), _p(dy), _dt(dy), _p(levels.table), _p(grid_grad), levels.n_params)
    return grid_grad


def sh_fwd(dirs, dtype=torch.float16):
    out = torch.empty((dirs.shape[0], 16), dtype=dtype, device=dirs.device)
    lib.call("ngp_sh_fwd", _stream(), dirs.shape[0], _p(dirs), F16 if dtype == torch.float16 else F32, _p(out))
    return out


def mlp_fwd(W, X, n_hidden_matmuls, save_inter=True):
    n = X.shape[0]
    inter = torch.empty(((n_hidden_matmuls + 1) * n, 64), dtype=torch.float16, device=X.device) if save_inter else None
    Y = torch.empty((n, 16), dtype=torch.float16, device=X.device)
    lib.call("ngp_mlp_fwd", _stream(), _p(W), _p(X), _p(inter), _p(Y), n_hidden_matmuls, n)
    return Y, inter


def mlp_bwd(W, X, inter, dY, n_hidden_matmuls, n_out_valid, need_dx=True, need_temps=False):
    n = X.shape[0]
    dX = torch.empty((n, 32), dtype=torch.float16, device=X.device) if need_dx else None
    temps = torch.empty(((n_hidden_matmuls + 1) * n, 64), dtype=torch.float16, device=X.device) if need_temps else None
    dW = torch.empty(W.numel(), dtype=torch.float32, device=X.device)
    lib.call("ngp_mlp_bwd", _stream(), _p(W), _p(X), _p(inter), _p(dY), _p(dX), _p(temps), _p(dW), n_hidden_matmuls, n_out_valid, n)
    return dX, temps, dW


def mlp_bwd_dgrad(W, inter, dY_feature_major, n_hidden_matmuls, need_dx=False):
    n = dY_feature_major.shape[1]
    dX = torch.empty((n, 32), dtype=torch.float16, device=W.device) if need_dx else None
    temps = torch.empty(((n_hidden_matmuls + 1) * n, 64), dtype=torch.float16, device=W.device)
    lib.call("ngp_mlp_bwd_dgrad", _stream(), _p(W), _p(inter), _p(dY_feature_major), _p(dX), _p(temps), n_hidden_matmuls, n)
    return dX, temps


def network_fwd(coords, grid, levels, wd, wr, n_dev=None, save_enc=True, out=None, enc=None):
    n = coords.shape[0]
    if out is None:
        out = torch.empty((n, 4), dtype=torch.float16, device=coords.device)
    if enc is None and save_enc:
        enc = torch.empty((n, 32), dtype=torch.float16, device=coords.device)
    lib.call("ngp_network_fwd", _stream(), n, _p(n_dev), _p(coords), _p(grid), _p(levels.table), _p(wd), _p(wr), _p(out), _p(enc))
    return out, enc


def network_bwd(coords, enc, levels, wd, wr, dout, grid_grad, dwd, dwr, n_dev=None):
    lib.call("ngp_network_bwd", _stream(), coords.shape[0], _p(n_dev), _p(coords), _p(enc), _p(levels.table), _p(wd), _p(wr), _p(dout),
             _p(grid_grad), _p(dwd), _p(dwr))


def density_fwd(pos, grid, levels, wd):
    out = torch.empty(pos.shape[0], dtype=torch.float16, device=pos.device)
    lib.call("ngp_density_fwd", _stream(), pos.shape[0], _p(pos), _p(grid), _p(levels.table), _p(wd), _p(out))
    return out


def _mesh_workspace(device, n=0, n_verts=0, n_tris=0):
    b = np.zeros(1, np.uint64)
    lib.call("ngp_mesh_workspace_bytes", int(n), int(n_verts), int(n_tris), b.ctypes.data)
    return torch.empty(max(int(b[0]), 1), dtype=torch.uint8, device=device)


def density_lattice(n, grid, levels, wd):
    if not 2 <= int(n) <= 1024:
        raise lib.NgpError(f"density_lattice: resolution {n} is outside [2, 1024]")
    field = torch.empty((n, n, n), dtype=torch.float32, device=grid.device)
    lib.call("ngp_density_lattice", _stream(), int(n), _p(grid), _p(levels.table), _p(wd), _p(field))
    return field


def marching_cubes(field, iso=0.5, workspace=None):
    import ctypes
    n = field.shape[0]
    assert field.dim() == 3 and field.shape == (n, n, n) and field.dtype == torch.float32
    if workspace is None:
        workspace = _mesh_workspace(field.device, n=n)
    counts = np.zeros(2, np.uint64)
    cp = counts.ctypes.data_as(ctypes.c_void_p)
    lib.call("ngp_marching_cubes", _stream(), n, _p(field), float(iso), _p(workspace), None, 0, None, 0, cp)
    V, T = int(counts[0]), int(counts[1])
    verts = torch.empty((V, 3), dtype=torch.float32, device=field.device)
    tris = torch.empty((T, 3), dtype=torch.int32, device=field.device)
    if T or V:
        lib.call("ngp_marching_cubes", _stream(), n, _p(field), float(iso), _p(workspace), _p(verts), V, _p(tris), T, cp)
    return verts, tris


def mesh_largest_component(verts, tris, workspace=None):
    import ctypes
    V, T = verts.shape[0], tris.shape[0]
    if workspace is None:
        workspace = _mesh_workspace(verts.device, n_verts=V, n_tris=T)
    vo = torch.empty_like(verts)
    to = torch.empty_like(tris)
    counts = np.zeros(2, np.uint64)
    lib.call("ngp_mesh_largest_component", _stream(), V, T, _p(verts), _p(tris), _p(workspace), _p(vo), _p(to), counts.ctypes.data_as(ctypes.c_void_p))
    return vo[:int(counts[0])], to[:int(counts[1])]


def mesh_vertex_normals(verts, tris, workspace=None):
    V, T = verts.shape[0], tris.shape[0]
    if workspace is None:
        workspace = _mesh_workspace(verts.device, n_verts=V, n_tris=T)
    normals = torch.empty_like(verts)
    lib.call("ngp_mesh_vertex_normals", _stream(), V, T, _p(verts), _p(tris) if T else None, _p(workspace), _p(normals))
    return normals


RENDER_CAPACITY = 1 << 22
RENDER_MAX_K = 64


def render_k_steps(capacity, n_alive):
    return max(1, min(RENDER_MAX_K, int(capacity) // max(int(n_alive), 1)))


def render_workspace_layout(n_rays, capacity):
    lay = np.zeros(4, np.uint64)
    lib.call("ngp_render_workspace_bytes", int(n_rays), int(capacity), lay.ctypes.data)
    return tuple(int(x) for x in lay)


def render_workspace(n_rays, workspace=None, capacity=RENDER_CAPACITY):
    nbytes = render_workspace_layout(n_rays, capacity)[0]
    if workspace is not None and workspace.numel() >= nbytes:
        return workspace
    return torch.empty(max(nbytes, 1), dtype=torch.uint8, device="cuda")


def render_rays(rays_o, rays_d, bitfield, aabb, cone_angle, near, cascades, const_dt, rng, grid, levels, wd, wr, jitter_tile,
                min_transmittance=0.0, capacity=RENDER_CAPACITY, workspace=None):
    import ctypes
    R, dev = rays_o.shape[0], rays_o.device
    nbytes, off_rows, off_net, off_cnt = render_workspace_layout(R, capacity)
    if workspace is None or workspace.numel() < nbytes:
        workspace = torch.empty(max(nbytes, 1), dtype=torch.uint8, device=dev)
    rows = workspace[off_rows:off_rows + 28 * capacity].view(torch.float32).view(capacity, 7)
    net = workspace[off_net:off_net + 8 * capacity].view(torch.float16).view(capacity, 4)
    n_rows = workspace[off_cnt:off_cnt + 4].view(torch.int32)
    rgb = torch.empty((R, 3), dtype=torch.float32, device=dev)
    alpha = torch.empty((R, 1), dtype=torch.float32, device=dev)
    n_samples = torch.empty(R, dtype=torch.int32, device=dev)
    alive = np.zeros(1, np.uint32)
    ap = alive.ctypes.data_as(ctypes.c_void_p)
    lib.call("ngp_render_init", _stream(), R, int(capacity), _p(workspace), float(aabb[0]), float(aabb[1]), _p(rays_o), _p(rays_d), float(cone_angle),
             float(near), int(cascades), int(const_dt), int(rng[0]), int(rng[1]), int(jitter_tile), _p(rgb), _p(alpha), _p(n_samples), ap)
    rounds = 0
    while int(alive[0]):
        n_alive = int(alive[0])
        k = render_k_steps(capacity, n_alive)
        lib.call("ngp_render_march_round", _stream(), R, int(capacity), _p(workspace), n_alive, k, float(aabb[0]), float(aabb[1]), _p(rays_o),
                 _p(rays_d), _p(bitfield), float(cone_angle), int(cascades), int(const_dt))
        bound = min(n_alive, int(capacity) // k) * k
        network_fwd(rows[:bound], grid, levels, wd, wr, n_dev=n_rows, save_enc=False, out=net[:bound])
        lib.call("ngp_render_composite_round", _stream(), R, int(capacity), _p(workspace), n_alive, k, float(min_transmittance), int(cascades),
                 _p(rgb), _p(alpha), _p(n_samples), ap)
        rounds += 1
    return rgb, alpha, n_samples, rounds


def march(rays_o, rays_d, bitfield, aabb, max_samples, cone_angle, near, cascades, const_dt, rng, coords=None, workspace=None):
    R = rays_o.shape[0]
    dev = rays_o.device
    counters = torch.empty(2, dtype=torch.int32, device=dev)
    ray_idx = torch.zeros(R, dtype=torch.int32, device=dev)
    numsteps = torch.empty((R, 2), dtype=torch.int32, device=dev)
    if coords is None:
        coords = torch.empty((max_samples, 7), dtype=torch.float32, device=dev)
    if workspace is None:
        workspace = torch.empty(int(lib.load().ngp_march_workspace_bytes(R)), dtype=torch.uint8, device=dev)
    lib.call("ngp_march", _stream(), R, float(aabb[0]), float(aabb[1]), max_samples, _p(rays_o), _p(rays_d), _p(bitfield), float(cone_angle),
             float(near), cascades, int(const_dt), int(rng[0]), int(rng[1]), _p(counters), _p(ray_idx), _p(numsteps), _p(coords), _p(workspace))
    return coords, ray_idx, numsteps, counters


def compact(coords, numsteps, max_compacted, alias=False, zero_fill=True):
    R = numsteps.shape[0]
    dev = coords.device
    out = coords if alias else torch.empty((max_compacted, 7), dtype=torch.float32, device=dev)
    ns = torch.empty((R, 2), dtype=torch.int32, device=dev)
    counters = torch.empty(2, dtype=torch.int32, device=dev)
    lib.call("ngp_compact", _stream(), R, max_compacted, _p(coords), _p(numsteps), _p(out), _p(ns), _p(counters), int(zero_fill))
    return out, ns, counters


def composite_fwd(net, coords, numsteps_in, numsteps_c, bg, cascades=5):
    R = numsteps_c.shape[0]
    rgb = torch.empty((R, 3), dtype=torch.float32, device=net.device)
    lib.call("ngp_composite_fwd", _stream(), R, _p(net), _dt(net), _p(coords), _p(numsteps_in), _p(numsteps_c), _p(bg), cascades, _p(rgb))
    return rgb


def composite_bwd(net, coords, numsteps_c, loss_grad, rgb_ray, mean, cascades=5):
    R = numsteps_c.shape[0]
    dnet = torch.empty_like(net)
    lib.call("ngp_composite_bwd", _stream(), R, net.shape[0], _p(net), _dt(net), _p(coords), _p(numsteps_c), _p(loss_grad), _p(rgb_ray), _p(mean),
             cascades, _p(dnet))
    return dnet


def composite_infer(net, coords, numsteps, cascades=5):
    R = numsteps.shape[0]
    rgb = torch.empty((R, 3), dtype=torch.float32, device=net.device)
    alpha = torch.empty((R, 1), dtype=torch.float32, device=net.device)
    lib.call("ngp_composite_infer", _stream(), R, _p(net), _dt(net), _p(coords), _p(numsteps), cascades, _p(rgb), _p(alpha))
    return rgb, alpha


def composite_loss_bwd(net, coords, numsteps_in, numsteps_c, bg, target, mean, delta=0.1, cascades=5, dnet=None, rgb=None, loss=None, reg_scale=1.0):
    R = numsteps_c.shape[0]
    dev = net.device
    if dnet is None:
        dnet = torch.zeros_like(net)
    if rgb is None:
        rgb = torch.empty((R, 3), dtype=torch.float32, device=dev)
    if loss is None:
        loss = torch.empty(R, dtype=torch.float32, device=dev)
    lib.call("ngp_composite_loss_bwd", _stream(), R, net.shape[0], _p(net), _p(coords), _p(numsteps_in), _p(numsteps_c), _p(bg), _p(target),
             float(delta), _p(mean), cascades, _p(rgb), _p(loss), _p(dnet), float(reg_scale))
    return rgb, loss, dnet


def grid_mark_untrained(grid, focal, xforms, res):
    lib.call("ngp_grid_mark_untrained", _stream(), grid.numel(), _p(grid), xforms.shape[0], _p(focal), _p(xforms), int(res[0]), int(res[1]))


def grid_generate_samples(n, rng, step_dev, aabb, grid, n_cascades, thresh):
    pos = torch.empty((n, 3), dtype=torch.float32, device=grid.device)
    idx = torch.empty(n, dtype=torch.int32, device=grid.device)
    lib.call("ngp_grid_generate_samples", _stream(), n, int(rng[0]), int(rng[1]), _p(step_dev), float(aabb[0]), float(aabb[1]), _p(grid), _p(pos),
             _p(idx), n_cascades, float(thresh))
    return pos, idx


def grid_splat(indices, mlp_out, grid_tmp):
    lib.call("ngp_grid_splat", _stream(), indices.numel(), _p(indices), _p(mlp_out), _dt(mlp_out), _p(grid_tmp))


def grid_ema(grid, grid_tmp, decay=0.95):
    lib.call("ngp_grid_ema", _stream(), grid.numel(), float(decay), _p(grid), _p(grid_tmp))


def grid_update_bitfield(grid, mean, bitfield, cascades=5):
    lib.call("ngp_grid_update_bitfield", _stream(), _p(grid), _p(mean), _p(bitfield), cascades)


def adam_ema(param, grad, m, v, master, lr, step, beta1=0.9, beta2=0.99, eps=1e-15, ema_decay=0.95, grad_scale=1.0, zero_grad=True):
    lib.call("ngp_adam_ema", _stream(), param.numel(), _p(param), _dt(param), _p(grad), _dt(grad), float(grad_scale), _p(m), _p(v), _p(master),
             float(lr), float(beta1), float(beta2), float(eps), int(step), float(ema_decay), int(zero_grad))


def raygen(pix, W, H, xforms, focal, principal):
    n = pix.numel()
    dev = pix.device
    img = torch.empty(n, dtype=torch.int32, device=dev)
    o = torch.empty((n, 3), dtype=torch.float32, device=dev)
    d = torch.empty((n, 3), dtype=torch.float32, device=dev)
    lib.call("ngp_raygen", _stream(), n, _p(pix), W, H, _p(xforms), _p(focal), _p(principal), _p(img), _p(o), _p(d))
    return img, o, d


def prepare_batch(pix, W, H, xforms, focal, principal, images, bg):
    n = pix.numel()
    dev = pix.device
    img = torch.empty(n, dtype=torch.int32, device=dev)
    o = torch.empty((n, 3), dtype=torch.float32, device=dev)
    d = torch.empty((n, 3), dtype=torch.float32, device=dev)
    target = torch.empty((n, 3), dtype=torch.float32, device=dev)
    lib.call("ngp_prepare_batch", _stream(), n, _p(pix), W, H, _p(xforms), _p(focal), _p(principal), _p(images), int(images.dtype == torch.uint8),
             _p(bg), _p(img), _p(o), _p(d), _p(target))
    return img, o, d, target


def blend_target(rgba, bg, target=None):
    n = rgba.shape[0]
    if target is None:
        target = torch.empty((n, 3), dtype=torch.float32, device=rgba.device)
    lib.call("ngp_blend_target", _stream(), n, _p(rgba), _p(bg), _p(target))
    return target


def step_state_new(device="cuda"):
    return torch.zeros(int(lib.load().ngp_step_state_bytes()), dtype=torch.uint8, device=device)


def step_state_set(state, rng, pix_cursor, adam_steps_done, lr, beta1=0.9, beta2=0.99, eps=1e-15, ema_decay=0.95, grad_scale=1.0):
    lib.call("ngp_step_state_set", _stream(), _p(state), int(rng[0]), int(rng[1]), int(pix_cursor), int(adam_steps_done), float(lr), float(beta1),
             float(beta2), float(eps), float(ema_decay), float(grad_scale))


def step_state_tick(state, pix_advance, lr, beta1=0.9, beta2=0.99, eps=1e-15, ema_decay=0.95, grad_scale=1.0):
    lib.call("ngp_step_state_tick", _stream(), _p(state), int(pix_advance), float(lr), float(beta1), float(beta2), float(eps), float(ema_decay),
             float(grad_scale))


def prepare_batch_dev(n, pix_list, state, pix_offset, W, H, xforms, focal, principal, images, bg):
    dev = pix_list.device
    img = torch.empty(n, dtype=torch.int32, device=dev)
    o = torch.empty((n, 3), dtype=torch.float32, device=dev)
    d = torch.empty((n, 3), dtype=torch.float32, device=dev)
    target = torch.empty((n, 3), dtype=torch.float32, device=dev)
    lib.call("ngp_prepare_batch_dev", _stream(), n, _p(pix_list), _p(state), int(pix_offset), W, H, _p(xforms), _p(focal), _p(principal), _p(images),
             int(images.dtype == torch.uint8), _p(bg), _p(img), _p(o), _p(d), _p(target))
    return img, o, d, target


def march_dev(rays_o, rays_d, bitfield, aabb, max_samples, cone_angle, near, cascades, const_dt, state, ray_offset=0, coords=None, workspace=None):
    R = rays_o.shape[0]
    dev = rays_o.device
    counters = torch.empty(2, dtype=torch.int32, device=dev)
    ray_idx = torch.zeros(R, dtype=torch.int32, device=dev)
    numsteps = torch.empty((R, 2), dtype=torch.int32, device=dev)
    if coords is None:
        coords = torch.empty((max_samples, 7), dtype=torch.float32, device=dev)
    if workspace is None:
        workspace = torch.empty(int(lib.load().ngp_march_workspace_bytes(R)), dtype=torch.uint8, device=dev)
    lib.call("ngp_march_dev", _stream(), R, float(aabb[0]), float(aabb[1]), max_samples, _p(rays_o), _p(rays_d), _p(bitfield), float(cone_angle),
             float(near), cascades, int(const_dt), _p(state), int(ray_offset), _p(counters), _p(ray_idx), _p(numsteps), _p(coords), _p(workspace))
    return coords, ray_idx, numsteps, counters


def adam_ema_dev(param, grad, m, v, master, state, zero_grad=True):
    lib.call("ngp_adam_ema_dev", _stream(), param.numel(), _p(param), _dt(param), _p(grad), _dt(grad), _p(m), _p(v), _p(master), _p(state), int(zero_grad))


def pcg32_seed(seed=1337, seq=1):
    si = np.zeros(2, np.uint64)
    lib.load().ngp_pcg32_seed(seed, seq, si.ctypes.data)
    return si


def pcg32_advance(si, delta=1 << 32):
    lib.load().ngp_pcg32_advance(si.ctypes.data, delta)
    return si


def dp_exchange_step(world, rank, slice_len, n_w, peer_table, peer_table_grad, peer_w_grad, peer_flags, epoch, m, v, master, w_param, w_m, w_v,
                     w_master, lr, step, beta1=0.9, beta2=0.99, eps=1e-15, ema_decay=0.95, grad_scale=1.0):
    import ctypes
    assert m.numel() == slice_len and v.numel() == slice_len and master.numel() == slice_len and w_param.numel() == n_w
    lib.call("ngp_dp_exchange_step", _stream(), int(world), int(rank), int(slice_len), int(n_w), ctypes.addressof(peer_table),
             ctypes.addressof(peer_table_grad), ctypes.addressof(peer_w_grad), ctypes.addressof(peer_flags), int(epoch), _p(m), _p(v), _p(master),
             _p(w_param), _p(w_m), _p(w_v), _p(w_master), float(grad_scale), float(lr), float(beta1), float(beta2), float(eps), int(step),
             float(ema_decay))


def dp_exchange_wait(world, my_flags, epoch):
    lib.call("ngp_dp_exchange_wait", _stream(), int(world), _p(my_flags), int(epoch))
```

### jnerf_b200/runner.py

```python
import contextlib
import os

import numpy as np
import torch

from . import dp, ops
from .plugin import losses as L
from .utils.config import get_cfg
from .utils.registry import DATASETS, LOSSES, NETWORKS, OPTIMS, SAMPLERS, build_from_cfg


class Runner:
    def __init__(self, rank=0, world_size=1, process_group=None):
        self.cfg = get_cfg()
        cfg = self.cfg
        self.rank, self.world_size, self.pg = rank, world_size, process_group
        self.dataset = {"train": build_from_cfg(cfg.dataset.train, DATASETS)}
        cfg.dataset_obj = self.dataset["train"]
        self.dataset["val"] = build_from_cfg(cfg.dataset.val, DATASETS) if cfg.dataset.val else self.dataset["train"]
        self.dataset["test"] = None
        self.model = build_from_cfg(cfg.model, NETWORKS)
        cfg.model_obj = self.model
        self.sampler = build_from_cfg(cfg.sampler, SAMPLERS)
        cfg.sampler_obj = self.sampler
        if world_size > 1:
            self.sampler.dp_group = (process_group, world_size)
        params = list(self.model.parameters())
        self.optimizer = build_from_cfg(cfg.optim, OPTIMS, params=params)
        self.optimizer = build_from_cfg(cfg.expdecay, OPTIMS, nested_optimizer=self.optimizer)
        self.ema_optimizer = build_from_cfg(cfg.ema, OPTIMS, params=params)
        self.ema_optimizer.attach(self.optimizer)
        self.loss_func = build_from_cfg(cfg.loss, LOSSES)
        self.background_color = cfg.background_color
        self.tot_train_steps = cfg.tot_train_steps
        self.n_rays_per_batch = cfg.n_rays_per_batch
        self.W, self.H = self.dataset["train"].resolution
        self.start = 0
        cfg.m_training_step = 0
        self.val_freq = 4096
        self.fast = bool(getattr(self.model, "fused", False))
        self._table_work, self._pending_epoch = None, None
        self._host_stage = None
        self._render_ws = None
        self._dev_state = None
        self._pipe = None
        self._st = {id(s.p): s for s in self.optimizer._nested_optimizer.state}
        if world_size > 1 and not self.fast:
            raise ValueError("data-parallel training needs the fused model (fp16=True, use_fully=True): the per-operator autograd step "
                             "shards the ray batch but has no gradient exchange, the replicas would silently diverge")
        if self.fast:
            self._init_fast_path()
        self._bg_gen = torch.Generator(device="cuda").manual_seed(int(cfg.seed or 1) + 7)

    def _init_fast_path(self):
        dev = "cuda"
        m = self.model
        cap = self.sampler.target_batch_size
        self.grid_grad = torch.zeros(m.pos_encoder.m_grid.numel(), dtype=torch.float16, device=dev)
        n_w = m.density_mlp.con_weights.numel() + m.rgb_mlp.con_weights.numel()
        self.w_grad = torch.zeros(n_w + 8, dtype=torch.float32, device=dev)
        self.dwd = self.w_grad[:m.density_mlp.con_weights.numel()]
        self.dwr = self.w_grad[m.density_mlp.con_weights.numel():n_w]
        self.net_out = torch.zeros((cap, 4), dtype=torch.float16, device=dev)
        self.enc = torch.empty((cap, 32), dtype=torch.float16, device=dev)
        self.dnet = torch.zeros((cap, 4), dtype=torch.float16, device=dev)
        self.last_loss = None
        self.last_rgb = None
        if self.world_size == 1:
            self._dev_state = ops.step_state_new()
            self._dev_expect = None
            self._graphs, self._graph_seen, self._graph_pool, self._cap_stream = {}, {}, None, None
            self._graphs_enabled = os.environ.get("NGP_GRAPHS", "0") == "1" and torch.cuda.is_available() and hasattr(torch.cuda, "CUDAGraph")
            self.graph_replays = 0
            self._graph_after = int(os.environ.get("NGP_GRAPH_AFTER", "20"))
        if os.environ.get("NGP_PIPELINE", "1") == "1" and not getattr(self, "_graphs_enabled", False):
            at = os.environ.get("NGP_PIPE_AT", "front")
            assert at in ("front", "fwd", "bwd")
            raw = self.sampler._coords_raw
            self._pipe = dict(stream=torch.cuda.Stream(), coords=[torch.zeros_like(raw), torch.zeros_like(raw)], made=0, pending=None, at=at, mid=torch.cuda.Event(),
                              back_done=[torch.cuda.Event(), torch.cuda.Event()], prefetched=0, aux=torch.cuda.Stream(),
                              bwd_done=torch.cuda.Event(), aux_done=torch.cuda.Event(), main=None)
        if self.world_size > 1:
            self._init_sharded_table()

    def _init_sharded_table(self):
        import os
        g = self.model.pos_encoder.m_grid
        m = self.model
        n, W = g.numel(), self.world_size
        mode = os.environ.get("NGP_DP_EXCHANGE", "auto")
        assert mode in ("auto", "p2p", "nccl")
        self.dp_mode = "p2p" if mode == "p2p" or (mode == "auto" and dp.peer_exchange_available(W)) else "nccl"
        P = dp.padded_len(n, W)
        nd, nr = m.density_mlp.con_weights.numel(), m.rgb_mlp.con_weights.numel()
        if self.dp_mode == "p2p":
            try:
                self._arena = dp.PeerArena(n, nd + nr, W, self.rank, self.pg)
            except RuntimeError as e:
                if mode == "p2p":
                    raise
                if self.rank == 0:
                    print(f"[jnerf_b200] peer-memory exchange unavailable ({e}); using the NCCL exchange", flush=True)
                self.dp_mode = "nccl"
        if self.dp_mode == "p2p":
            self._table, self._table_grad, self.w_grad = self._arena.table, self._arena.table_grad, self._arena.w_grad
            self.dwd, self.dwr = self.w_grad[:nd], self.w_grad[nd:nd + nr]
            self._peers = {k: self._arena.peers(k) for k in ("table", "table_grad", "w_grad", "flags")}
            self._w_param = torch.cat([m.density_mlp.con_weights.data.reshape(-1), m.rgb_mlp.con_weights.data.reshape(-1)]).contiguous()
            m.density_mlp.con_weights.data = self._w_param[:nd].view_as(m.density_mlp.con_weights.data)
            m.rgb_mlp.con_weights.data = self._w_param[nd:].view_as(m.rgb_mlp.con_weights.data)
            std, str_ = self._st[id(m.density_mlp.con_weights)], self._st[id(m.rgb_mlp.con_weights)]
            self._w_m, self._w_v = torch.cat([std.m, str_.m]), torch.cat([std.v, str_.v])
            self._w_master = torch.cat([std.master, str_.master])
            for st, lo_, hi_ in ((std, 0, nd), (str_, nd, nd + nr)):
                st.m, st.v, st.master = self._w_m[lo_:hi_], self._w_v[lo_:hi_], self._w_master[lo_:hi_]
            self._epoch, self._pending_epoch = 0, None
        else:
            self._table = torch.zeros(P, dtype=g.dtype, device=g.device)
            self._table_grad = torch.zeros(P, dtype=self.grid_grad.dtype, device=g.device)
        self._table[:n].copy_(g.data.reshape(-1))
        g.data = self._table[:n]
        self.grid_grad = self._table_grad[:n]
        self._lo, self._hi = dp.slice_bounds(P, W, self.rank)
        self._slice_grad = torch.empty(self._hi - self._lo, dtype=self.grid_grad.dtype, device=g.device)
        self._slice_param = self._table[self._lo:self._hi].clone()
        st = self._st[id(g)]
        master = torch.zeros(P, dtype=torch.float32, device=g.device)
        master[:n].copy_(st.master)
        st.master = master[self._lo:self._hi].clone()
        st.m = torch.zeros(self._hi - self._lo, dtype=torch.float32, device=g.device)
        st.v = torch.zeros_like(st.m)

    def _table_ready(self, zero_on=None):
        if self._table_work is not None:
            self._table_work.wait()
            self._table_work = None
        if getattr(self, "_pending_epoch", None) is not None:
            ops.dp_exchange_wait(self.world_size, self._arena.flags, self._pending_epoch)
            self._pending_epoch = None
            if zero_on is None:
                self._arena.grads.zero_()
                return False
            stream, ev = zero_on
            ev.record(torch.cuda.current_stream())
            stream.wait_event(ev)
            with torch.cuda.stream(stream):
                self._arena.grads.zero_()
                ev.record(stream)
            return True
        return False

    def _gather_table_state(self):
        g = self.model.pos_encoder.m_grid
        st, n = self._st[id(g)], g.numel()
        out = []
        for t in (st.m, st.v, st.master):
            full = torch.empty(self._table.numel(), dtype=torch.float32, device=g.device)
            dp.all_gather_slices(full, t, self.pg, self.world_size)
            out.append(full[:n].clone())
        return out

    def _scatter_table_state(self, m, v, master):
        g = self.model.pos_encoder.m_grid
        st, n = self._st[id(g)], g.numel()
        for dst, src in ((st.m, m), (st.v, v), (st.master, master)):
            full = torch.zeros(self._table.numel(), dtype=torch.float32, device=g.device)
            full[:n].copy_(src.reshape(-1))
            dst.copy_(full[self._lo:self._hi])

    def next_batch(self):
        ds = self.dataset["train"]
        n = self.sampler.n_rays_per_batch
        pix = ds.next_pixels(n * self.world_size)
        if self.world_size > 1:
            pix = pix[self.rank * n:(self.rank + 1) * n]
        img_ids, rays_o, rays_d = ds.rays_for(pix)
        return img_ids, rays_o, rays_d, ds.rgba_for(pix)

    def _lr_for_step(self, k):
        dec = self.optimizer
        f = dec.m_learning_rate_factor
        for q in range(dec.steps, k + 1):
            if q >= dec.decay_start and (q - dec.decay_start) % dec.decay_interval == 0 and q <= dec.decay_end:
                f *= dec.decay_base
        return dec.base_lr * f

    def _step_body(self, R, lr_next):
        s, m, ds, st = self.sampler, self.model, self.dataset["train"], self._dev_state
        adam = self.optimizer._nested_optimizer
        bg = torch.rand((R, 3), device="cuda", generator=self._bg_gen)
        img_ids, rays_o, rays_d, target = ops.prepare_batch_dev(R, ds.shuffle_index, st, 0, ds.W, ds.H, ds.transforms_gpu, ds.focal_lengths,
                                                                ds.principal, ds.image_data, bg)
        s.sample_dev(rays_o, rays_d, st)
        coords, n_dev = s.coords_compacted, s.n_samples_dev
        self.net_forward(coords, n_dev)
        rgb, loss, _ = ops.composite_loss_bwd(self.net_out, coords, s._rays_numsteps, s._rays_numsteps_compacted, bg, target,
                                              s.density_grid_mean, delta=self.loss_func.delta, cascades=s.NERF_CASCADES, dnet=self.dnet)
        self.net_backward(coords, n_dev)
        for p, g in ((m.pos_encoder.m_grid, self.grid_grad), (m.density_mlp.con_weights, self.dwd), (m.rgb_mlp.con_weights, self.dwr)):
            stp = self._st[id(p)]
            ops.adam_ema_dev(p.data, g, stp.m, stp.v, stp.master, st, zero_grad=True)
        ops.step_state_tick(st, R, lr_next, adam.betas[0], adam.betas[1], adam.eps, self.ema_optimizer.decay, 1.0)
        self.last_loss, self.last_rgb = loss, rgb
        return loss

    def _train_step_dev(self):
        cfg, s, ds = self.cfg, self.sampler, self.dataset["train"]
        adam, dec = self.optimizer._nested_optimizer, self.optimizer
        i = cfg.m_training_step
        R = s.n_rays_per_batch
        edge = i % s.update_den_freq == 0 or i % s.update_den_freq == s.update_den_freq - 1
        if i % s.update_den_freq == 0:
            s.update_density_grid()
        if R > s._march_ws_rays:
            s._ensure_march_ws(2 * R)
            self._graphs.clear()
            self._graph_pool = None
        start = ds.reserve_pixels(R)
        lr, lr_next = self._lr_for_step(dec.steps), self._lr_for_step(dec.steps + 1)
        want = (int(s.rng[0]), int(s.rng[1]), start, adam.n_step, lr)
        if self._dev_expect != want:
            ops.step_state_set(self._dev_state, s.rng, start, adam.n_step, lr, adam.betas[0], adam.betas[1], adam.eps, self.ema_optimizer.decay, 1.0)
        key = (R, lr_next)
        g = self._graphs.get(key) if self._graphs_enabled and not edge else None
        if g is not None:
            g[0].replay()
            ops.lib.launch_count += g[1]
            self.graph_replays += 1
            loss = g[2]
            self.last_loss, self.last_rgb = g[2], g[3]
            s._rays_numsteps, s._rays_numsteps_compacted, s._counters_compacted, s._coords = g[4]
        else:
            seen = self._graph_seen.get(key, 0) + 1
            self._graph_seen[key] = seen
            if self._graphs_enabled and not edge and seen >= self._graph_after and len(self._graphs) < 64:
                graph = torch.cuda.CUDAGraph()
                if hasattr(graph, "register_generator_state"):
                    graph.register_generator_state(self._bg_gen)
                n0 = ops.lib.launch_count
                if self._cap_stream is None:
                    self._cap_stream = torch.cuda.Stream()
                main = torch.cuda.current_stream()
                self._cap_stream.wait_stream(main)
                with torch.cuda.stream(self._cap_stream):
                    if self._graph_pool is None:
                        graph.capture_begin(capture_error_mode="thread_local")
                    else:
                        graph.capture_begin(pool=self._graph_pool, capture_error_mode="thread_local")
                    loss = self._step_body(R, lr_next)
                    graph.capture_end()
                main.wait_stream(self._cap_stream)
                if self._graph_pool is None:
                    self._graph_pool = graph.pool()
                self._graphs[key] = (graph, ops.lib.launch_count - n0, loss, self.last_rgb,
                                     (s._rays_numsteps, s._rays_numsteps_compacted, s._counters_compacted, s._coords))
                ops.lib.launch_count = n0
                graph.replay()
                ops.lib.launch_count += self._graphs[key][1]
                self.graph_replays += 1
            else:
                loss = self._step_body(R, lr_next)
        ops.pcg32_advance(s.rng)
        dec.advance_lr()
        adam.n_step += 1
        self.ema_optimizer.steps += 1
        self._dev_expect = (int(s.rng[0]), int(s.rng[1]), start + R, adam.n_step, lr_next)
        if i % s.update_den_freq == s.update_den_freq - 1:
            s.update_batch_rays()
        cfg.m_training_step = i + 1
        return loss

    def _front(self, step, batch, prefetch):
        P, s, ds = self._pipe, self.sampler, self.dataset["train"]
        slot = P["made"] & 1
        main = P["main"] if P["main"] is not None else torch.cuda.current_stream()
        side = P["stream"]
        if prefetch:
            side.wait_event(P["mid"])
        (side if prefetch else main).wait_event(P["back_done"][slot])
        with (torch.cuda.stream(side) if prefetch else contextlib.nullcontext()):
            rng_before = s.rng.copy()
            W = self.world_size
            if step % s.update_den_freq == 0:
                assert not prefetch
                self._table_ready()
                s.update_density_grid()
            if batch is None:
                R = s.n_rays_per_batch
                pix = ds.next_pixels(R * W)
                bg = torch.rand((R * W, 3), device="cuda", generator=self._bg_gen)
                if W > 1:
                    lo, hi = dp.shard_range(R, self.rank)
                    pix, bg = pix[lo:hi], bg[lo:hi]
                bg = bg.contiguous()
                img_ids, rays_o, rays_d, target = ops.prepare_batch(pix.contiguous(), ds.W, ds.H, ds.transforms_gpu, ds.focal_lengths,
                                                                    ds.principal, ds.image_data, bg)
            else:
                img_ids, rays_o, rays_d, rgba = batch
                R = rays_o.shape[0]
                bg = torch.rand((R * W, 3), device="cuda", generator=self._bg_gen)
                if W > 1:
                    bg = bg[self.rank * R:(self.rank + 1) * R]
                bg = bg.contiguous()
                target = ops.blend_target(rgba.contiguous(), bg)
            numsteps, ns_c, cnt_c, coords = s.sample_front(rays_o, rays_d, P["coords"][slot], ray_index_offset=dp.shard_range(R, self.rank)[0])
            done = torch.cuda.Event()
            done.record(side if prefetch else main)
        P["made"] += 1
        P["prefetched"] += int(prefetch)
        return dict(step=step, src=batch, slot=slot, bg=bg, target=target, numsteps=numsteps, ns_c=ns_c, cnt_c=cnt_c, coords=coords, done=done,
                    rng_before=rng_before, rays=(img_ids, rays_o, rays_d), side=prefetch)

    def _adapt_ray_batch(self, F):
        P, s = self._pipe, self.sampler
        side = P["stream"]
        if P.get("count_host") is None:
            P["count_host"], P["count_ev"] = torch.zeros(1, dtype=torch.int32).pin_memory(), torch.cuda.Event()
        side.wait_event(F["done"])
        with torch.cuda.stream(side):
            if self.world_size > 1:
                dp.global_sum_count(s.measured_batch_size, self.pg, self.world_size)
            P["count_host"].copy_(s.measured_batch_size, non_blocking=True)
            s.measured_batch_size.zero_()
            P["count_ev"].record(side)
        P["count_ev"].synchronize()
        P["main"].wait_event(P["count_ev"])
        s.update_batch_rays(measured_total=int(P["count_host"][0]))

    def _sync_front(self):
        P = self._pipe
        if P is not None and P["pending"] is not None:
            torch.cuda.current_stream().wait_event(P["pending"]["done"])

    def _train_step_pipe(self, batch=None, next_batch=None):
        cfg, s, P = self.cfg, self.sampler, self._pipe
        i = cfg.m_training_step
        main = P["main"] = torch.cuda.current_stream()
        F, P["pending"] = P["pending"], None
        if F is not None and (F["step"] != i or F["src"] is not batch):
            main.wait_event(F["done"])
            F = None
        if F is None:
            F = self._front(i, batch, prefetch=False)
        elif F["side"]:
            main.wait_event(F["done"])
        if P["at"] == "front":
            P["mid"].record(main)
        s.__dict__.update(_rays_numsteps=F["numsteps"], _rays_numsteps_compacted=F["ns_c"], _counters_compacted=F["cnt_c"], _coords=F["coords"])
        coords, n_dev = F["coords"], F["cnt_c"][0:1]
        zeroing = self._table_ready(zero_on=(P["aux"], P["aux_done"]))
        self.net_forward(coords, n_dev)
        if P["at"] == "fwd":
            P["mid"].record(main)
        rgb, loss, _ = ops.composite_loss_bwd(self.net_out, coords, F["numsteps"], F["ns_c"], F["bg"], F["target"], s.density_grid_mean,
                                              delta=self.loss_func.delta, cascades=s.NERF_CASCADES, dnet=self.dnet,
                                              reg_scale=float(self.world_size))
        if zeroing:
            main.wait_event(P["aux_done"])
        self.net_backward(coords, n_dev)
        if P["at"] == "bwd":
            P["mid"].record(main)
        lr = self.optimizer.advance_lr()
        adam = self.optimizer._nested_optimizer
        adam.n_step += 1
        self.ema_optimizer.steps += 1
        m = self.model
        hyper = (lr, adam.n_step, adam.betas[0], adam.betas[1], adam.eps, self.ema_optimizer.decay)
        if self.world_size > 1:
            self._optimizer_step(lr, adam.n_step)
            return self._pipe_finish(F, loss, rgb, batch, next_batch)
        P["bwd_done"].record(main)
        P["aux"].wait_event(P["bwd_done"])
        with torch.cuda.stream(P["aux"]):
            for p_, g_ in ((m.density_mlp.con_weights, self.dwd), (m.rgb_mlp.con_weights, self.dwr)):
                st = self._st[id(p_)]
                ops.adam_ema(p_.data, g_, st.m, st.v, st.master, *hyper, grad_scale=1.0, zero_grad=True)
            P["aux_done"].record(P["aux"])
        st = self._st[id(m.pos_encoder.m_grid)]
        ops.adam_ema(m.pos_encoder.m_grid.data, self.grid_grad, st.m, st.v, st.master, *hyper, grad_scale=1.0, zero_grad=True)
        main.wait_event(P["aux_done"])
        return self._pipe_finish(F, loss, rgb, batch, next_batch)

    def _pipe_finish(self, F, loss, rgb, batch, next_batch):
        cfg, s, P = self.cfg, self.sampler, self._pipe
        i = cfg.m_training_step
        P["back_done"][F["slot"]].record(P["main"])
        self.last_loss, self.last_rgb = loss, rgb
        cfg.m_training_step = i + 1
        self._pipe_last = F
        if i % s.update_den_freq == s.update_den_freq - 1:
            self._adapt_ray_batch(F)
        if (i + 1) % s.update_den_freq != 0 and (batch is None or next_batch is not None):
            P["pending"] = self._front(i + 1, next_batch if batch is not None else None, prefetch=True)
        return loss

    def train_step(self, batch=None, next_batch=None):
        if self._pipe is not None:
            return self._train_step_pipe(batch, next_batch)
        if batch is None and self._dev_state is not None:
            return self._train_step_dev()
        cfg, s, m = self.cfg, self.sampler, self.model
        i = cfg.m_training_step
        if batch is None:
            ds = self.dataset["train"]
            R = s.n_rays_per_batch
            pix = ds.next_pixels(R * self.world_size)
            bg = torch.rand((R * self.world_size, 3), device="cuda", generator=self._bg_gen)
            if self.world_size > 1:
                lo, hi = dp.shard_range(R, self.rank)
                pix, bg = pix[lo:hi], bg[lo:hi]
            img_ids, rays_o, rays_d, target = ops.prepare_batch(pix.contiguous(), ds.W, ds.H, ds.transforms_gpu, ds.focal_lengths, ds.principal,
                                                                ds.image_data, bg.contiguous())
        else:
            img_ids, rays_o, rays_d, rgba = batch
            R = rays_o.shape[0]
            bg = torch.rand((R * self.world_size, 3), device="cuda", generator=self._bg_gen)
            if self.world_size > 1:
                bg = bg[self.rank * R:(self.rank + 1) * R].contiguous()
            target = ops.blend_target(rgba.contiguous(), bg.contiguous())
        if i % s.update_den_freq == 0:
            self._table_ready()
        s.sample(img_ids, rays_o, rays_d, is_training=True, ray_index_offset=dp.shard_range(R, self.rank)[0])
        self._table_ready()
        coords, n_dev = s.coords_compacted, s.n_samples_dev
        self.net_forward(coords, n_dev)
        rgb, loss, _ = ops.composite_loss_bwd(self.net_out, coords, s._rays_numsteps, s._rays_numsteps_compacted, bg, target.contiguous(),
                                              s.density_grid_mean, delta=self.loss_func.delta, cascades=s.NERF_CASCADES, dnet=self.dnet,
                                              reg_scale=float(self.world_size))
        self.net_backward(coords, n_dev)
        lr = self.optimizer.advance_lr()
        adam = self.optimizer._nested_optimizer
        adam.n_step += 1
        self.ema_optimizer.steps += 1
        self._optimizer_step(lr, adam.n_step)
        self.last_loss, self.last_rgb = loss, rgb
        cfg.m_training_step = i + 1
        return loss

    def train_step_host(self, batch, next_batch=None):
        st = self._host_stage
        if st is None:
            st = self._host_stage = dict(stream=torch.cuda.Stream(), slots=[None, None], ready=[torch.cuda.Event(), torch.cuda.Event()],
                                         free=[torch.cuda.Event(), torch.cuda.Event()], staged=[None, None], dev=[None, None], k=0,
                                         loss_host=torch.zeros(1, dtype=torch.float32).pin_memory(), done=torch.cuda.Event())
            for e in st["free"]:
                e.record()
        main = torch.cuda.current_stream()

        def put(b, slot):
            R = b[1].shape[0]
            if st["slots"][slot] is None or st["slots"][slot][1].shape[0] < R:
                cap = max(2 * R, 4096)
                st["slots"][slot] = (torch.empty(cap, dtype=torch.int32, device="cuda"), torch.empty((cap, 3), device="cuda"),
                                     torch.empty((cap, 3), device="cuda"), torch.empty((cap, 4), device="cuda"))
            with torch.cuda.stream(st["stream"]):
                st["stream"].wait_event(st["free"][slot])
                for dst, src in zip(st["slots"][slot], b):
                    dst[:R].copy_(src, non_blocking=True)
                st["ready"][slot].record()
            st["staged"][slot] = (b, R)
            st["dev"][slot] = tuple(t[:R] for t in st["slots"][slot])

        slot = st["k"] % 2
        if st["staged"][slot] is None or st["staged"][slot][0] is not batch:
            put(batch, slot)
        if next_batch is not None:
            put(next_batch, 1 - slot)
        main.wait_event(st["ready"][slot])
        dev, nxt = st["dev"][slot], None
        if next_batch is not None and self._pipe is not None:
            nxt = st["dev"][1 - slot]
            self._pipe["stream"].wait_event(st["ready"][1 - slot])
        loss = self.train_step(dev, nxt)
        st["free"][slot].record(main)
        st["staged"][slot] = None
        st["k"] += 1
        st["done"].record(main)
        with torch.cuda.stream(st["stream"]):
            st["stream"].wait_event(st["done"])
            loss.record_stream(st["stream"])
            st["loss_host"].copy_(loss.mean().reshape(1), non_blocking=True)
        return st["loss_host"]

    def net_forward(self, coords, n_dev):
        m = self.model
        ops.network_fwd(coords, m.pos_encoder.m_grid, m.pos_encoder.levels, m.density_mlp.con_weights, m.rgb_mlp.con_weights,
                        n_dev=n_dev, out=self.net_out, enc=self.enc)

    def net_backward(self, coords, n_dev):
        m = self.model
        ops.network_bwd(coords, self.enc, m.pos_encoder.levels, m.density_mlp.con_weights, m.rgb_mlp.con_weights, self.dnet,
                        self.grid_grad, self.dwd, self.dwr, n_dev=n_dev)

    def _optimizer_step(self, lr, n_step):
        m = self.model
        adam = self.optimizer._nested_optimizer
        hyper = (lr, n_step, adam.betas[0], adam.betas[1], adam.eps, self.ema_optimizer.decay)
        if self.world_size > 1 and self.dp_mode == "p2p":
            st = self._st[id(m.pos_encoder.m_grid)]
            self._epoch += 1
            ops.dp_exchange_step(self.world_size, self.rank, self._hi - self._lo, self._w_param.numel(), self._peers["table"],
                                 self._peers["table_grad"], self._peers["w_grad"], self._peers["flags"], self._epoch, st.m, st.v, st.master,
                                 self._w_param, self._w_m, self._w_v, self._w_master, *hyper, grad_scale=1.0 / self.world_size)
            self._pending_epoch = self._epoch
            return
        if self.world_size > 1:
            dp.reduce_scatter_sum(self._slice_grad, self._table_grad, self.pg, self.world_size, self.rank)
            scale = dp.allreduce_grads((self.w_grad,), self.pg, self.world_size)
            st = self._st[id(m.pos_encoder.m_grid)]
            ops.adam_ema(self._slice_param, self._slice_grad, st.m, st.v, st.master, *hyper, grad_scale=scale, zero_grad=False)
            self._table_work = dp.all_gather_slices(self._table, self._slice_param, self.pg, self.world_size, async_op=True)
            self._table_grad.zero_()
            tensors = ((m.density_mlp.con_weights, self.dwd), (m.rgb_mlp.con_weights, self.dwr))
        else:
            scale = 1.0
            tensors = ((m.pos_encoder.m_grid, self.grid_grad), (m.density_mlp.con_weights, self.dwd), (m.rgb_mlp.con_weights, self.dwr))
        for p, g in tensors:
            st = self._st[id(p)]
            ops.adam_ema(p.data, g, st.m, st.v, st.master, *hyper, grad_scale=scale, zero_grad=True)

    def train_step_autograd(self, batch=None):
        cfg = self.cfg
        i = cfg.m_training_step
        img_ids, rays_o, rays_d, rgba = self.next_batch() if batch is None else batch
        bg = torch.rand((rays_o.shape[0], 3), device="cuda", generator=self._bg_gen)
        target = (rgba[:, :3] * rgba[:, 3:] + bg * (1 - rgba[:, 3:])).detach()
        pos, dir_ = self.sampler.sample(img_ids, rays_o, rays_d, is_training=True)
        network_outputs = self.model(pos, dir_)
        rgb = self.sampler.rays2rgb(network_outputs, bg)
        loss = self.loss_func(rgb, target)
        self.optimizer.step(loss)
        self.ema_optimizer.ema_step()
        cfg.m_training_step = i + 1
        return loss.sum(-1)

    def train(self, steps=None, log_every=0):
        end = self.tot_train_steps if steps is None else self.cfg.m_training_step + steps
        step_fn = self.train_step if self.fast else self.train_step_autograd
        while self.cfg.m_training_step < end:
            loss = step_fn()
            i = self.cfg.m_training_step
            if log_every and i % log_every == 0 and self.rank == 0:
                print(f"STEP={i} | LOSS={loss.mean().item():.6f} | rays/batch={self.sampler.n_rays_per_batch}", flush=True)

    @torch.no_grad()
    def render_img(self, dataset_mode="train", img_id=0):
        self._table_ready()
        self._sync_front()
        ds = self.dataset[dataset_mode]
        W, H = ds.resolution
        rays_o, rays_d = ds.generate_rays_total_test(img_id)
        tile = self.cfg.n_rays_per_batch
        img = torch.empty((H * W, 3), device="cuda")
        alpha = torch.empty((H * W, 1), device="cuda")
        ids = torch.zeros(tile, dtype=torch.int32, device="cuda")
        s, m = self.sampler, self.model
        for p in range(0, H * W, tile):
            e = min(p + tile, H * W)
            o, d = rays_o[p:e], rays_d[p:e]
            if e - p < tile:
                o = torch.cat([o, torch.ones((tile - (e - p), 3), device="cuda")])
                d = torch.cat([d, torch.ones((tile - (e - p), 3), device="cuda")])
            s.sample(ids, o.contiguous(), d.contiguous())
            coords = s._coords
            if self.fast:
                out, _ = ops.network_fwd(coords.contiguous(), m.pos_encoder.m_grid, m.pos_encoder.levels, m.density_mlp.con_weights,
                                         m.rgb_mlp.con_weights, save_enc=False) if coords.shape[0] else (torch.empty((0, 4), dtype=torch.float16, device="cuda"), None)
            else:
                out = m(coords[:, :3], coords[:, 4:])
            rgb, a = s.rays2rgb(out, inference=True)
            img[p:e], alpha[p:e] = rgb[:e - p], a[:e - p]
        bgc = torch.tensor(self.background_color, dtype=torch.float32, device="cuda")
        img = img + bgc * (1 - alpha)
        tar = ds.rgba_for(torch.arange(H * W, device="cuda", dtype=torch.int32) + int(img_id) * H * W)
        tar = tar[:, :3] * tar[:, 3:] + bgc * (1 - tar[:, 3:])
        return img.reshape(H, W, 3), tar.reshape(H, W, 3)

    @torch.no_grad()
    def render_img_nosync(self, dataset_mode="train", img_id=0):
        assert self.fast, "render_img_nosync drives the fused network kernel"
        self._table_ready()
        self._sync_front()
        ds = self.dataset[dataset_mode]
        W, H = ds.resolution
        rays_o, rays_d = ds.generate_rays_total_test(img_id)
        tile = self.cfg.n_rays_per_batch
        n_pix = H * W
        n_pad = (n_pix + tile - 1) // tile * tile
        if n_pad > n_pix:
            fill = torch.ones((n_pad - n_pix, 3), device="cuda")
            rays_o, rays_d = torch.cat([rays_o, fill]), torch.cat([rays_d, fill])
        img = torch.empty((n_pad, 3), device="cuda")
        alpha = torch.empty((n_pad, 1), device="cuda")
        s, m = self.sampler, self.model
        if getattr(self, "_infer_net_out", None) is None:
            self._infer_net_out = torch.empty((s.max_samples, 4), dtype=torch.float16, device="cuda")
        s._ensure_march_ws(tile)
        for p in range(0, n_pad, tile):
            coords, _, numsteps, counters = ops.march(
                rays_o[p:p + tile].contiguous(), rays_d[p:p + tile].contiguous(), s.density_grid_bitfield, s.aabb_range, s.max_samples,
                s.cone_angle_constant, s.near_distance, s.NERF_CASCADES, s.const_dt, s.rng, coords=s._coords_raw, workspace=s._march_ws)
            ops.pcg32_advance(s.rng)
            ops.network_fwd(coords, m.pos_encoder.m_grid, m.pos_encoder.levels, m.density_mlp.con_weights, m.rgb_mlp.con_weights,
                            n_dev=counters[1:2], save_enc=False, out=self._infer_net_out)
            rgb, a = ops.composite_infer(self._infer_net_out, coords, numsteps, s.NERF_CASCADES)
            img[p:p + tile], alpha[p:p + tile] = rgb, a
        bgc = torch.tensor(self.background_color, dtype=torch.float32, device="cuda")
        img = img[:n_pix] + bgc * (1 - alpha[:n_pix])
        tar = ds.rgba_for(torch.arange(n_pix, device="cuda", dtype=torch.int32) + int(img_id) * n_pix)
        tar = tar[:, :3] * tar[:, 3:] + bgc * (1 - tar[:, 3:])
        return img.reshape(H, W, 3), tar.reshape(H, W, 3)

    @torch.no_grad()
    def render_rays(self, rays_o, rays_d, min_transmittance=1e-4):
        assert self.fast, "render_rays drives the fused network kernel"
        self._table_ready()
        self._sync_front()
        s, m = self.sampler, self.model
        R, tile = rays_o.shape[0], int(self.cfg.n_rays_per_batch)
        self._render_ws = ops.render_workspace(R, self._render_ws)
        out = ops.render_rays(rays_o.contiguous(), rays_d.contiguous(), s.density_grid_bitfield, s.aabb_range, s.cone_angle_constant, s.near_distance,
                              s.NERF_CASCADES, s.const_dt, s.rng, m.pos_encoder.m_grid, m.pos_encoder.levels, m.density_mlp.con_weights,
                              m.rgb_mlp.con_weights, tile, min_transmittance=min_transmittance, workspace=self._render_ws)
        ops.pcg32_advance(s.rng, ((R + tile - 1) // tile) << 32)
        return out

    def release_render_workspace(self):
        self._render_ws = None

    def _render_frame(self, rays_o, rays_d, W, H, min_transmittance):
        rgb, alpha, n, rounds = self.render_rays(rays_o, rays_d, min_transmittance)
        if not getattr(self.cfg, "alpha_image", False):
            rgb = rgb + torch.tensor(self.background_color, dtype=torch.float32, device=rgb.device) * (1 - alpha)
        return rgb.reshape(H, W, 3), alpha.reshape(H, W, 1), n.reshape(H, W), rounds

    def pose_rays(self, pose):
        from .plugin.dataset import matrix_nerf2ngp
        ds = self.dataset["train"]
        W, H = ds.resolution
        xf = matrix_nerf2ngp(np.asarray(pose, np.float32)[:3, :4], ds.scale, ds.offset, getattr(ds, "correct_pose", (1, -1, -1)))
        dev = ds.transforms_gpu.device
        xforms = torch.from_numpy(np.ascontiguousarray(xf.T).reshape(1, 12)).to(dev)
        pix = torch.arange(H * W, dtype=torch.int32, device=dev)
        _, o, d = ops.raygen(pix, W, H, xforms, ds.focal_lengths[:1].contiguous(), ds.principal[:1].contiguous())
        return o, d

    @torch.no_grad()
    def render_img_with_pose(self, pose, min_transmittance=1e-4):
        W, H = self.dataset["train"].resolution
        o, d = self.pose_rays(pose)
        return self._render_frame(o, d, W, H, min_transmittance)[0]

    def _save_path(self):
        return os.path.join(self.cfg.log_dir or ".", self.cfg.exp_name or "exp")

    @staticmethod
    def save_img(path, img, alpha=None):
        from PIL import Image
        img = img.detach().cpu().numpy() if torch.is_tensor(img) else np.asarray(img)
        if alpha is not None:
            alpha = alpha.detach().cpu().numpy() if torch.is_tensor(alpha) else np.asarray(alpha)
            img = np.concatenate([img, alpha], axis=-1)
        Image.fromarray((img * 255 + 0.5).clip(0, 255).astype(np.uint8)).save(path)

    @torch.no_grad()
    def render(self, save_path=None, load_ckpt=False, min_transmittance=1e-4):
        try:
            import cv2
        except ImportError as e:
            raise RuntimeError("Runner.render writes the video with OpenCV: install opencv-python (cv2) to use it") from e
        from .utils.camera_path import path_spherical
        if load_ckpt:
            self.load_ckpt(self.cfg.ckpt_path)
        if not save_path:
            save_path = os.path.join(self._save_path(), "demo.mp4")
        elif not str(save_path).endswith(".mp4"):
            raise ValueError(f"Runner.render: the video path must end in .mp4, got {save_path}")
        os.makedirs(os.path.dirname(os.path.abspath(save_path)), exist_ok=True)
        W, H = self.dataset["train"].resolution
        writer = cv2.VideoWriter(str(save_path), cv2.VideoWriter_fourcc(*"mp4v"), 28, (W, H))
        try:
            for pose in path_spherical():
                img = self.render_img_with_pose(pose, min_transmittance)
                u8 = (img.cpu().numpy() * 255 + 0.5).clip(0, 255).astype(np.uint8)
                writer.write(np.ascontiguousarray(u8[..., ::-1]))
        finally:
            writer.release()
            self.release_render_workspace()
        return save_path

    @torch.no_grad()
    def render_test(self, save_img=True, save_path=None, min_transmittance=1e-4):
        ds = self.dataset["test"]
        save_path = self._save_path() if save_path is None else save_path
        if save_img:
            os.makedirs(save_path, exist_ok=True)
        exp = self.cfg.exp_name
        W, H = ds.resolution
        bgc = torch.tensor(self.background_color, dtype=torch.float32, device=ds.transforms_gpu.device)
        have_img = getattr(ds, "have_img", True)
        mse = []
        for i in range(ds.n_images):
            o, d = ds.generate_rays_total_test(i)
            img, alpha, _, _ = self._render_frame(o, d, W, H, min_transmittance)
            if save_img:
                self.save_img(os.path.join(save_path, f"{exp}_r_{i}.png"), img, alpha if getattr(self.cfg, "alpha_image", False) else None)
            if not have_img:
                continue
            tar = ds.rgba_for(torch.arange(H * W, device=bgc.device, dtype=torch.int32) + i * H * W)
            tar = (tar[:, :3] * tar[:, 3:] + bgc * (1 - tar[:, 3:])).reshape(H, W, 3)
            if save_img:
                self.save_img(os.path.join(save_path, f"{exp}_gt_{i}.png"), tar)
            mse.append(float(L.img2mse(img, tar).item()))
        return mse

    @torch.no_grad()
    def test(self, load_ckpt=False, min_transmittance=1e-4):
        if load_ckpt:
            self.load_ckpt(self.cfg.ckpt_path)
        if self.dataset["test"] is None:
            self.dataset["test"] = build_from_cfg(self.cfg.dataset.test, DATASETS)
        try:
            mse = self.render_test(save_path=os.path.join(self._save_path(), "test"), min_transmittance=min_transmittance)
        finally:
            self.release_render_workspace()
        if not getattr(self.dataset["test"], "have_img", True):
            return None
        psnr = sum(float(L.mse2psnr(torch.tensor(v)).item()) for v in mse) / len(mse)
        print(f"TOTAL TEST PSNR===={psnr}", flush=True)
        return psnr

    @torch.no_grad()
    def extract_mesh(self, out_dir, resolution=512):
        import os
        from .utils.ply import write_ply
        assert self.fast, "extract_mesh drives the fused network kernels"
        self._table_ready()
        self._sync_front()
        N = int(resolution)
        if not 2 <= N <= 1024:
            raise ValueError(f"extract_mesh: resolution {N} is outside [2, 1024]")
        os.makedirs(out_dir, exist_ok=True)
        s, m = self.sampler, self.model
        ev = [torch.cuda.Event(enable_timing=True) for _ in range(6)]
        ev[0].record()
        field = ops.density_lattice(N, m.pos_encoder.m_grid, m.pos_encoder.levels, m.density_mlp.con_weights)
        ev[1].record()
        verts0, tris0 = ops.marching_cubes(field, 0.5)
        ev[2].record()
        del field
        v0_host, t0_host = verts0.cpu().numpy(), tris0.cpu().numpy()
        write_ply(os.path.join(out_dir, "mesh-origin.ply"), v0_host, t0_host)
        ev[3].record()
        verts, tris = ops.mesh_largest_component(verts0, tris0)
        normals = ops.mesh_vertex_normals(verts, tris)
        ev[4].record()
        perm = torch.tensor([1, 0, 2], device=verts.device)
        v_model, n_model = verts[:, perm], normals[:, perm]
        zero = (n_model == 0).all(dim=1, keepdim=True)
        dirs = torch.where(zero, torch.tensor([0.0, 0.0, -1.0], device=verts.device), -n_model).contiguous()
        origins = (v_model - 0.2 * dirs).contiguous()
        V = verts.shape[0]
        tile = self.cfg.n_rays_per_batch
        rgb = torch.empty((V, 3), device=verts.device)
        alpha = torch.empty((V, 1), device=verts.device)
        if getattr(self, "_infer_net_out", None) is None:
            self._infer_net_out = torch.empty((s.max_samples, 4), dtype=torch.float16, device="cuda")
        s._ensure_march_ws(tile)
        for p in range(0, V, tile):
            coords, _, numsteps, counters = ops.march(
                origins[p:p + tile].contiguous(), dirs[p:p + tile].contiguous(), s.density_grid_bitfield, s.aabb_range, s.max_samples,
                s.cone_angle_constant, s.near_distance, s.NERF_CASCADES, s.const_dt, s.rng, coords=s._coords_raw, workspace=s._march_ws)
            ops.pcg32_advance(s.rng)
            ops.network_fwd(coords, m.pos_encoder.m_grid, m.pos_encoder.levels, m.density_mlp.con_weights, m.rgb_mlp.con_weights,
                            n_dev=counters[1:2], save_enc=False, out=self._infer_net_out)
            c, a = ops.composite_infer(self._infer_net_out, coords, numsteps, s.NERF_CASCADES)
            rgb[p:p + tile], alpha[p:p + tile] = c, a
        ev[5].record()
        img = rgb.cpu().numpy().astype(np.float64) + np.asarray(self.background_color, np.float64) * (1 - alpha.cpu().numpy().astype(np.float64))
        colors = (img * 255 + 0.5).clip(0, 255).astype(np.uint8)
        v_host, t_host = verts.cpu().numpy(), tris.cpu().numpy()
        write_ply(os.path.join(out_dir, "mesh-color.ply"), v_host, t_host, colors)
        torch.cuda.synchronize()
        names = ("density_lattice", "marching_cubes", "write_origin", "component_normals", "colour")
        times = {k: round(ev[i].elapsed_time(ev[i + 1]), 3) for i, k in enumerate(names)}
        return dict(vertices=v_host, triangles=t_host, normals=normals.cpu().numpy(), colors=colors, origins=origins.cpu().numpy(),
                    dirs=dirs.cpu().numpy(), n_verts_origin=int(v0_host.shape[0]), n_tris_origin=int(t0_host.shape[0]),
                    n_verts=int(v_host.shape[0]), n_tris=int(t_host.shape[0]), stage_ms=times)

    @torch.no_grad()
    def psnr(self, dataset_mode="val", max_images=None):
        ds = self.dataset[dataset_mode]
        n = ds.n_images if max_images is None else min(max_images, ds.n_images)
        tot = 0.0
        for k in range(n):
            img, tar = self.render_img(dataset_mode, k)
            tot += float(L.mse2psnr(L.img2mse(img, tar)).item())
        return tot / n

    def save_ckpt(self, path):
        adam = self.optimizer._nested_optimizer
        self._table_ready()
        nested = adam.state_dict()
        if self.world_size > 1:
            k = [id(s.p) for s in adam.state].index(id(self.model.pos_encoder.m_grid))
            full = self._gather_table_state()
            for key, t in zip(("m", "v", "master"), full):
                nested[key] = list(nested[key])
                nested[key][k] = t
            if self.rank != 0:
                return
        sampler_state = self.sampler.state_dict()
        if self._pipe is not None and self._pipe["pending"] is not None:
            sampler_state["rng"] = torch.from_numpy(self._pipe["pending"]["rng_before"].astype(np.int64))
        ck = {"global_step": self.cfg.m_training_step, "model": self.model.state_dict(), "sampler": sampler_state,
              "optimizer": self.optimizer.state_dict(), "nested_optimizer": nested, "ema_optimizer": self.ema_optimizer.state_dict()}
        if str(path).endswith(".pkl") and not hasattr(self.model.density_mlp, "con_weights"):
            raise NotImplementedError("the .pkl interchange format is written for the fused-MLP parameter layout (con_weights); "
                                      "save the nn.Linear fallback model to a .pt path")
        if str(path).endswith(".pkl"):
            from .utils import ckpt_compat as cc
            dec = self.optimizer
            ref = cc.native_to_reference(
                ck, adam_hyper=dict(lr=adam.lr, eps=adam.eps, betas=tuple(adam.betas)),
                expdecay_hyper=dict(base_lr=dec.base_lr, decay_start=dec.decay_start, decay_interval=dec.decay_interval, decay_base=dec.decay_base,
                                    decay_end=dec.decay_end),
                param_dtype=np.float16 if self.model.pos_encoder.m_grid.dtype == torch.float16 else np.float32)
            cc.write_reference_ckpt(ref, path)
            return
        torch.save(ck, path)

    def load_ckpt(self, path):
        self._table_ready()
        if self._pipe is not None:
            self._sync_front()
            self._pipe["pending"] = None
        if self.world_size > 1:
            import torch.distributed as dist
            dist.barrier(group=self.pg)
        if str(path).endswith(".pkl") and not hasattr(self.model.density_mlp, "con_weights"):
            raise NotImplementedError("the .pkl interchange format carries the fused-MLP parameter layout; load a .pt checkpoint instead")
        if str(path).endswith(".pkl"):
            from .utils import ckpt_compat as cc
            ck = cc.load_native_from_reference_file(path, self.model.pos_encoder.m_grid.numel(), "cuda",
                                                    {k: v.dtype for k, v in self.model.state_dict().items()})
        else:
            ck = torch.load(path, map_location="cuda", weights_only=True)
        self.cfg.m_training_step = self.start = ck["global_step"]
        self.model.load_state_dict(ck["model"])
        self.sampler.load_state_dict(ck["sampler"])
        self.optimizer.load_state_dict(ck["optimizer"])
        nested = ck["nested_optimizer"]
        if self.world_size > 1:
            adam = self.optimizer._nested_optimizer
            k = [id(s.p) for s in adam.state].index(id(self.model.pos_encoder.m_grid))
            self._scatter_table_state(nested["m"][k], nested["v"][k], nested["master"][k])
            st = self._st[id(self.model.pos_encoder.m_grid)]
            nested = dict(nested, **{key: [t if j != k else getattr(st, key) for j, t in enumerate(nested[key])] for key in ("m", "v", "master")})
            self._slice_param.copy_(self._table[self._lo:self._hi])
        self.optimizer._nested_optimizer.load_state_dict(nested)
        self.ema_optimizer.load_state_dict(ck["ema_optimizer"])


def lego_cfg(fp16=True, synthetic=True, **over):
    ds_type = "SyntheticNerfDataset" if synthetic else "NerfDataset"
    c = dict(
        sampler=dict(type="DensityGridSampler", update_den_freq=16),
        encoder=dict(pos_encoder=dict(type="HashEncoder"), dir_encoder=dict(type="SHEncoder")),
        model=dict(type="NGPNetworks", use_fully=True),
        loss=dict(type="HuberLoss", delta=0.1),
        optim=dict(type="Adam", lr=1e-1, eps=1e-15, betas=(0.9, 0.99)),
        ema=dict(type="EMA", decay=0.95),
        expdecay=dict(type="ExpDecay", decay_start=20_000, decay_interval=10_000, decay_base=0.33, decay_end=None),
        dataset=dict(train=dict(type=ds_type, root_dir="data/lego", batch_size=4096, mode="train"),
                     val=dict(type=ds_type, root_dir="data/lego", batch_size=4096, mode="val", preload_shuffle=False),
                     test=dict(type=ds_type, root_dir="data/lego", batch_size=4096, mode="test", preload_shuffle=False)),
        exp_name="lego", log_dir="./logs", tot_train_steps=40000, background_color=[0, 0, 0],
        hash_func="p0 ^ p1 * 19349663 ^ p2 * 83492791", cone_angle_constant=0.00390625, near_distance=0.2, n_rays_per_batch=4096,
        n_training_steps=16, target_batch_size=1 << 18, const_dt=True, load_ckpt=False, ckpt_path=None, alpha_image=False, fp16=fp16,
    )
    c.update(over)
    return c


def fox_cfg(fp16=True, synthetic=True, **over):
    c = lego_cfg(fp16=fp16, synthetic=synthetic)
    ds_type = "SyntheticNerfDataset" if synthetic else "NerfDataset"
    extra = dict(style="fox") if synthetic else {}
    c.update(dataset=dict(train=dict(type=ds_type, root_dir="data/fox", batch_size=4096, mode="train", **extra),
                          test=dict(type=ds_type, root_dir="data/fox", batch_size=4096, mode="test", preload_shuffle=False, **extra)),
             exp_name="fox", const_dt=False)
    c.update(over)
    return c
```

Before: 3.080 million.

## Fuse gradient flush, weight-grad reduce and Adam into one sweep kernel

The backward pass now writes its fixed-point grid gradients and per-CTA weight-gradient partials straight into scratch that the caller owns. A new train_sweep kernel then reduces the weight partials, converts the fixed-point grid gradients, applies Adam with EMA, and zeroes the scratch, all in one pass. This replaces the separate wgrad_reduce, grid_grad_flush and three adam_ema launches, and removes the fp16 grid_grad round-trip through memory. The trade-off is that the fused path only runs on a single GPU, and the pipelined path loses the aux-stream overlap it used for the MLP weight updates.

```diff
diff --git a/include/ngp_b200.h b/include/ngp_b200.h
--- a/include/ngp_b200.h
+++ b/include/ngp_b200.h
@@ -41,6 +41,10 @@
 int ngp_network_bwd(void* stream, uint32_t n_max, const uint32_t* n_dev, const float* coords, const void* enc_save,
                     const void* levels_dev, const void* w_density, const void* w_rgb, const void* dout,
                     void* grid_grad, float* dw_density, float* dw_rgb);
+int ngp_network_bwd_fx_bytes(uint64_t n_entries, uint64_t* fx_bytes, uint64_t* part_bytes);
+int ngp_network_bwd_fx(void* stream, uint32_t n_max, const uint32_t* n_dev, const float* coords, const void* enc_save,
+                       const void* levels_dev, const void* w_density, const void* w_rgb, const void* dout, uint32_t n_entries,
+                       void* fx, uint64_t fx_bytes, float* w_part, uint64_t part_bytes);
 int ngp_density_fwd(void* stream, uint32_t n, const float* pos, const void* grid, const void* levels_dev,
                     const void* w_density, void* sigma_out);
 
@@ -97,6 +101,9 @@
 int ngp_adam_ema(void* stream, uint64_t n, void* param, int param_dtype, void* grad, int grad_dtype, float grad_scale,
                  float* m, float* v, float* master, float lr, float beta1, float beta2, float eps, uint32_t step,
                  float ema_decay, int zero_grad);
+int ngp_train_sweep(void* stream, uint64_t n_entries, void* table, float* m, float* v, float* master, void* fx, const float* w_part,
+                    uint32_t bwd_rows, void* w_density, float* wd_m, float* wd_v, float* wd_master, void* w_rgb, float* wr_m,
+                    float* wr_v, float* wr_master, float lr, float beta1, float beta2, float eps, uint32_t step, float ema_decay);
 
 int ngp_dp_exchange_step(void* stream, int world, int rank, uint64_t slice_len, uint32_t n_w, void* const* peer_table,
                          void* const* peer_table_grad, float* const* peer_w_grad, uint32_t* const* peer_flags, uint32_t epoch, float* m,
@@ -130,6 +137,9 @@
                   float* coords, void* workspace);
 int ngp_adam_ema_dev(void* stream, uint64_t n, void* param, int param_dtype, void* grad, int grad_dtype, float* m, float* v,
                      float* master, const void* state_dev, int zero_grad);
+int ngp_train_sweep_dev(void* stream, uint64_t n_entries, void* table, float* m, float* v, float* master, void* fx, const float* w_part,
+                        uint32_t bwd_rows, void* w_density, float* wd_m, float* wd_v, float* wd_master, void* w_rgb, float* wr_m,
+                        float* wr_v, float* wr_master, const void* state_dev);
 
 void ngp_pcg32_seed(uint64_t initstate, uint64_t initseq, uint64_t* state_inc);
 void ngp_pcg32_advance(uint64_t* state_inc, int64_t delta);
diff --git a/jnerf_b200/csrc/fused_net.cu b/jnerf_b200/csrc/fused_net.cu
--- a/jnerf_b200/csrc/fused_net.cu
+++ b/jnerf_b200/csrc/fused_net.cu
@@ -1,4 +1,5 @@
 #include "mlp_tc.cuh"
+#include "train_common.cuh"
 #include <cstdlib>
 #include <cstdio>
 #include <mutex>
@@ -8,10 +9,6 @@
 
 namespace {
 using namespace mlp;
-
-constexpr int WD_W0 = 0, WD_WOUT = 64 * 32, WD_N = 64 * 32 + 16 * 64;
-constexpr int WR_W0 = 0, WR_W1 = 64 * 32, WR_WOUT = 64 * 32 + 64 * 64, WR_N = 64 * 32 + 64 * 64 + 16 * 64;
-constexpr int W_PART = WD_N + WR_N;
 
 constexpr uint32_t G_ENC = 0, G_HD = 4, G_RIN = 12, G_H1 = 16, G_H2F = 4 , G_H2B = 24;
 constexpr uint32_t G_ENC1 = 24;
@@ -240,7 +237,6 @@
 static_assert(SmemBwd3::total <= 227 * 1024, "backward CTA does not fit");
 constexpr uint32_t B3_STAGE = 1, B3_FULL = 2, B3_EMPTY = 3;
 
-constexpr float FX_SCALE = 4294967296.0f, FX_INV = 1.0f / 4294967296.0f;
 __device__ __forceinline__ void red_add_fx(unsigned long long* p, float v) {
     const long long q = __float2ll_rn(fminf(fmaxf(v, -65504.f), 65504.f) * FX_SCALE);
     if (q) asm volatile("red.global.add.u64 [%0], %1;" ::"l"(__cvta_generic_to_global(p)), "l"((unsigned long long)q) : "memory");
@@ -563,6 +559,22 @@
     return 0;
 }
 
+int bwd_launch(cudaStream_t s, uint32_t n_max, const uint32_t* n_dev, const float* coords, const void* enc_save, const void* levels_dev,
+               const void* w_density, const void* w_rgb, const void* dout, void* grid_grad, float* dw_density, float* dw_rgb,
+               unsigned long long* fx, uint32_t fx_entries, float* w_part) {
+    static const uint32_t dbg = getenv("NGP_BWD_DEBUG") ? (uint32_t)atoi(getenv("NGP_BWD_DEBUG")) : 0u;
+    if (ngp_first_use((const void*)network_bwd256_kernel)) NGP_CHECK_CUDA(cudaFuncSetAttribute(network_bwd256_kernel, cudaFuncAttributeMaxDynamicSharedMemorySize, (int)SmemBwd3::total));
+    NgpTensorMap enc_map{};
+    static const bool no_tma = getenv("NGP_NO_TMA") != nullptr;
+    const uint32_t enc_tma = (!no_tma && ngp_make_rows32_tensormap(&enc_map, enc_save, n_max)) ? 1u : 0u;
+    network_bwd256_kernel<<<bwd_ctas(n_max), B3_THREADS, SmemBwd3::total, s>>>(n_max, n_dev, coords, (const __half*)enc_save, (const NgpLevel*)levels_dev,
+                                                                              (const __half*)w_density, (const __half*)w_rgb, (const __half*)dout,
+                                                                              (__half*)grid_grad, dw_density, dw_rgb, fx, fx_entries, w_part,
+                                                                              ngp_err_flag(), dbg, enc_map, enc_tma);
+    NGP_LAUNCH_CHECK();
+    return 0;
+}
+
 }
 
 extern "C" {
@@ -614,22 +626,13 @@
                     const void* w_density, const void* w_rgb, const void* dout, void* grid_grad, float* dw_density, float* dw_rgb) {
     if (n_max == 0) return 0;
     cudaStream_t s = (cudaStream_t)stream;
-    const uint32_t ntiles = (n_max + ROWS - 1) / ROWS;
-    static const uint32_t dbg = getenv("NGP_BWD_DEBUG") ? (uint32_t)atoi(getenv("NGP_BWD_DEBUG")) : 0u;
-    if (ngp_first_use((const void*)network_bwd256_kernel)) NGP_CHECK_CUDA(cudaFuncSetAttribute(network_bwd256_kernel, cudaFuncAttributeMaxDynamicSharedMemorySize, (int)SmemBwd3::total));
-    const uint32_t grid_dim = min((ntiles + 1) / 2, (uint32_t)ngp_num_sms());
-    NgpTensorMap enc_map{};
-    static const bool no_tma = getenv("NGP_NO_TMA") != nullptr;
-    const uint32_t enc_tma = (!no_tma && ngp_make_rows32_tensormap(&enc_map, enc_save, n_max)) ? 1u : 0u;
     BwdScratch* b = nullptr;
     if (int rc = bwd_scratch(s, levels_dev, &b)) return rc;
-    network_bwd256_kernel<<<grid_dim, B3_THREADS, SmemBwd3::total, s>>>(n_max, n_dev, coords, (const __half*)enc_save, (const NgpLevel*)levels_dev,
-                                                                       (const __half*)w_density, (const __half*)w_rgb, (const __half*)dout,
-                                                                       (__half*)grid_grad, dw_density, dw_rgb, b ? b->fx : nullptr,
-                                                                       b ? b->fx_entries : 0u, b ? b->part : nullptr, ngp_err_flag(), dbg, enc_map, enc_tma);
-    NGP_LAUNCH_CHECK();
+    if (int rc = bwd_launch(s, n_max, n_dev, coords, enc_save, levels_dev, w_density, w_rgb, dout, grid_grad, dw_density, dw_rgb, b ? b->fx : nullptr,
+                            b ? b->fx_entries : 0u, b ? b->part : nullptr))
+        return rc;
     if (b) {
-        wgrad_reduce_kernel<<<(W_PART + 255) / 256, 256, 0, s>>>(b->part, grid_dim, dw_density, dw_rgb);
+        wgrad_reduce_kernel<<<(W_PART + 255) / 256, 256, 0, s>>>(b->part, bwd_ctas(n_max), dw_density, dw_rgb);
         NGP_LAUNCH_CHECK();
         grid_grad_flush_kernel<<<ngp_num_sms() * 8, 256, 0, s>>>((const NgpLevel*)levels_dev, b->fx_entries, reinterpret_cast<longlong2*>(b->fx),
                                                                  (__half2*)grid_grad);
@@ -638,4 +641,21 @@
     return 0;
 }
 
-}
+int ngp_network_bwd_fx_bytes(uint64_t n_entries, uint64_t* fx_bytes, uint64_t* part_bytes) {
+    *fx_bytes = 16 * n_entries;
+    *part_bytes = sizeof(float) * W_PART * (uint64_t)ngp_num_sms();
+    return 0;
+}
+
+int ngp_network_bwd_fx(void* stream, uint32_t n_max, const uint32_t* n_dev, const float* coords, const void* enc_save, const void* levels_dev,
+                       const void* w_density, const void* w_rgb, const void* dout, uint32_t n_entries, void* fx, uint64_t fx_bytes,
+                       float* w_part, uint64_t part_bytes) {
+    NGP_REQUIRE(fx != nullptr && fx_bytes >= 16 * (uint64_t)n_entries, "ngp_network_bwd_fx: the fixed-point scratch must hold 16 bytes per table entry");
+    NGP_REQUIRE(w_part != nullptr && part_bytes >= sizeof(float) * W_PART * (uint64_t)ngp_num_sms(),
+                "ngp_network_bwd_fx: the weight-gradient slots are smaller than ngp_network_bwd_fx_bytes gives");
+    if (n_max == 0) return 0;
+    return bwd_launch((cudaStream_t)stream, n_max, n_dev, coords, enc_save, levels_dev, w_density, w_rgb, dout, nullptr, nullptr, nullptr,
+                      (unsigned long long*)fx, n_entries, w_part);
+}
+
+}
diff --git a/jnerf_b200/csrc/optimizer.cu b/jnerf_b200/csrc/optimizer.cu
--- a/jnerf_b200/csrc/optimizer.cu
+++ b/jnerf_b200/csrc/optimizer.cu
@@ -1,17 +1,8 @@
-#include "ngp_common.cuh"
+#include "train_common.cuh"
 #include <cmath>
 #include <cstring>
 
 namespace {
-
-__device__ __forceinline__ float adam_one(float g, float& m, float& v, float& master, const AdamArgs& a) {
-    g = __fmul_rn(g, a.grad_scale);
-    m = __fmaf_rn(a.b1, m, __fmul_rn(1.f - a.b1, g));
-    v = __fmaf_rn(a.b2, v, __fmul_rn(__fmul_rn(1.f - a.b2, g), g));
-    const float p = __fsub_rn(master, __fdiv_rn(__fmul_rn(m, a.step_size), __fadd_rn(sqrtf(v), a.eps)));
-    master = __fmul_rn(__fmaf_rn(1.f - a.decay, p, __fmul_rn(__fmul_rn(a.decay, master), a.debias_old)), a.debias_new);
-    return master;
-}
 
 template <typename PT, typename GT>
 __global__ void __launch_bounds__(256) adam_ema_kernel(uint64_t n, PT* __restrict__ param, GT* __restrict__ grad, float* __restrict__ m,
@@ -75,6 +66,76 @@
     }
 }
 
+constexpr uint32_t SWEEP_THREADS = 256, SWEEP_W_BLOCKS = (W_PART + SWEEP_THREADS - 1) / SWEEP_THREADS;
+struct SweepTensor { __half* param; float *m, *v, *master; };
+
+__device__ __forceinline__ float2 fx_grad(longlong2 q) {
+    if (!(q.x | q.y)) return make_float2(0.f, 0.f);
+    return __half22float2(__floats2half2_rn(__fmul_rn(__ll2float_rn(q.x), FX_INV), __fmul_rn(__ll2float_rn(q.y), FX_INV)));
+}
+
+__global__ void __launch_bounds__(SWEEP_THREADS) train_sweep_kernel(uint64_t n_entries, SweepTensor tab, longlong2* __restrict__ fx,
+                                                                    const float* __restrict__ part, uint32_t nparts, SweepTensor wd, SweepTensor wr,
+                                                                    AdamArgs a, const NgpStepState* __restrict__ st) {
+    if (st) a = st->adam;
+    if (blockIdx.x < SWEEP_W_BLOCKS) {
+        const uint32_t e = blockIdx.x * SWEEP_THREADS + threadIdx.x;
+        if (e >= (uint32_t)W_PART) return;
+        float a0 = 0.f, a1 = 0.f, a2 = 0.f, a3 = 0.f;
+        uint32_t k = 0;
+#pragma unroll 4
+        for (; k + 4 <= nparts; k += 4) {
+            a0 += part[(size_t)k * W_PART + e];
+            a1 += part[(size_t)(k + 1) * W_PART + e];
+            a2 += part[(size_t)(k + 2) * W_PART + e];
+            a3 += part[(size_t)(k + 3) * W_PART + e];
+        }
+        for (; k < nparts; ++k) a0 += part[(size_t)k * W_PART + e];
+        const float g = __fadd_rn(0.f, (a0 + a1) + (a2 + a3));
+        const bool d = e < (uint32_t)WD_N;
+        const uint32_t j = d ? e : e - WD_N;
+        float* wm = (d ? wd.m : wr.m) + j;
+        float* wv = (d ? wd.v : wr.v) + j;
+        float* ws = (d ? wd.master : wr.master) + j;
+        float m1 = *wm, v1 = *wv, s1 = *ws;
+        const float p = adam_one(g, m1, v1, s1, a);
+        *wm = m1; *wv = v1; *ws = s1;
+        (d ? wd.param : wr.param)[j] = __float2half_rn(p);
+        return;
+    }
+    constexpr int UNROLL = 4;
+    const uint64_t T = (uint64_t)(gridDim.x - SWEEP_W_BLOCKS) * SWEEP_THREADS;
+    const uint64_t g0 = (uint64_t)(blockIdx.x - SWEEP_W_BLOCKS) * SWEEP_THREADS + threadIdx.x;
+    for (uint64_t i0 = g0; i0 < n_entries; i0 += UNROLL * T) {
+        longlong2 q[UNROLL];
+        float2 mm[UNROLL], vv[UNROLL], ms[UNROLL];
+#pragma unroll
+        for (int u = 0; u < UNROLL; ++u) {
+            const uint64_t i = i0 + u * T;
+            if (i < n_entries) {
+                q[u] = fx[i];
+                mm[u] = reinterpret_cast<const float2*>(tab.m)[i];
+                vv[u] = reinterpret_cast<const float2*>(tab.v)[i];
+                ms[u] = reinterpret_cast<const float2*>(tab.master)[i];
+            }
+        }
+#pragma unroll
+        for (int u = 0; u < UNROLL; ++u) {
+            const uint64_t i = i0 + u * T;
+            if (i < n_entries) {
+                const float2 g = fx_grad(q[u]);
+                if (q[u].x | q[u].y) fx[i] = make_longlong2(0, 0);
+                const float px = adam_one(g.x, mm[u].x, vv[u].x, ms[u].x, a);
+                const float py = adam_one(g.y, mm[u].y, vv[u].y, ms[u].y, a);
+                reinterpret_cast<float2*>(tab.m)[i] = mm[u];
+                reinterpret_cast<float2*>(tab.v)[i] = vv[u];
+                reinterpret_cast<float2*>(tab.master)[i] = ms[u];
+                reinterpret_cast<__half2*>(tab.param)[i] = __floats2half2_rn(px, py);
+            }
+        }
+    }
+}
+
 __global__ void raygen_kernel(uint32_t n, const uint32_t* __restrict__ pix, uint32_t W, uint32_t H, const float* __restrict__ xforms,
                               const float* __restrict__ focal, const float* __restrict__ principal, uint32_t* __restrict__ img_id,
                               float* __restrict__ rays_o, float* __restrict__ rays_d) {
@@ -282,6 +343,35 @@
     return adam_launch(stream, n, param, param_dtype, grad, grad_dtype, m, v, master, AdamArgs{}, zero_grad, (const NgpStepState*)state_dev);
 }
 
+static int sweep_launch(void* stream, uint64_t n_entries, void* table, float* m, float* v, float* master, void* fx, const float* w_part,
+                        uint32_t bwd_rows, void* w_density, float* wd_m, float* wd_v, float* wd_master, void* w_rgb, float* wr_m, float* wr_v,
+                        float* wr_master, AdamArgs a, const NgpStepState* st) {
+    NGP_REQUIRE(fx != nullptr && w_part != nullptr, "ngp_train_sweep: the backward's fixed-point scratch and weight-gradient slots are required");
+    const uint32_t blocks = (uint32_t)std::max<uint64_t>(1, std::min<uint64_t>((n_entries + 4 * SWEEP_THREADS - 1) / (4 * SWEEP_THREADS),
+                                                                           (uint64_t)ngp_num_sms() * 32));
+    train_sweep_kernel<<<SWEEP_W_BLOCKS + blocks, SWEEP_THREADS, 0, (cudaStream_t)stream>>>(
+        n_entries, SweepTensor{(__half*)table, m, v, master}, (longlong2*)fx, w_part, bwd_ctas(bwd_rows),
+        SweepTensor{(__half*)w_density, wd_m, wd_v, wd_master}, SweepTensor{(__half*)w_rgb, wr_m, wr_v, wr_master}, a, st);
+    NGP_LAUNCH_CHECK();
+    return 0;
+}
+
+int ngp_train_sweep(void* stream, uint64_t n_entries, void* table, float* m, float* v, float* master, void* fx, const float* w_part,
+                    uint32_t bwd_rows, void* w_density, float* wd_m, float* wd_v, float* wd_master, void* w_rgb, float* wr_m, float* wr_v,
+                    float* wr_master, float lr, float beta1, float beta2, float eps, uint32_t step, float ema_decay) {
+    NGP_REQUIRE(step >= 1, "ngp_train_sweep: step is 1-based");
+    return sweep_launch(stream, n_entries, table, m, v, master, fx, w_part, bwd_rows, w_density, wd_m, wd_v, wd_master, w_rgb, wr_m, wr_v,
+                        wr_master, make_adam_args(lr, beta1, beta2, eps, step, ema_decay, 1.0f), nullptr);
+}
+
+int ngp_train_sweep_dev(void* stream, uint64_t n_entries, void* table, float* m, float* v, float* master, void* fx, const float* w_part,
+                        uint32_t bwd_rows, void* w_density, float* wd_m, float* wd_v, float* wd_master, void* w_rgb, float* wr_m, float* wr_v,
+                        float* wr_master, const void* state_dev) {
+    NGP_REQUIRE(state_dev != nullptr, "ngp_train_sweep_dev: state_dev is required");
+    return sweep_launch(stream, n_entries, table, m, v, master, fx, w_part, bwd_rows, w_density, wd_m, wd_v, wd_master, w_rgb, wr_m, wr_v,
+                        wr_master, AdamArgs{}, (const NgpStepState*)state_dev);
+}
+
 static AdamArgs make_adam_args(float lr, float beta1, float beta2, float eps, uint32_t step, float ema_decay, float grad_scale) {
     AdamArgs a;
     const double n1 = 1.0 - std::pow((double)beta1, (double)step), n2 = 1.0 - std::pow((double)beta2, (double)step);
diff --git a/jnerf_b200/csrc/train_common.cuh b/jnerf_b200/csrc/train_common.cuh
--- /dev/null
+++ b/jnerf_b200/csrc/train_common.cuh
@@ -0,0 +1,23 @@
+#pragma once
+#include "ngp_common.cuh"
+#include <algorithm>
+
+constexpr int WD_W0 = 0, WD_WOUT = 64 * 32, WD_N = 64 * 32 + 16 * 64;
+constexpr int WR_W0 = 0, WR_W1 = 64 * 32, WR_WOUT = 64 * 32 + 64 * 64, WR_N = 64 * 32 + 64 * 64 + 16 * 64;
+constexpr int W_PART = WD_N + WR_N;
+
+inline uint32_t bwd_ctas(uint32_t n_max) {
+    const uint32_t ntiles = (n_max + 127) / 128;
+    return std::min((ntiles + 1) / 2, (uint32_t)ngp_num_sms());
+}
+
+constexpr float FX_SCALE = 4294967296.0f, FX_INV = 1.0f / 4294967296.0f;
+
+__device__ __forceinline__ float adam_one(float g, float& m, float& v, float& master, const AdamArgs& a) {
+    g = __fmul_rn(g, a.grad_scale);
+    m = __fmaf_rn(a.b1, m, __fmul_rn(1.f - a.b1, g));
+    v = __fmaf_rn(a.b2, v, __fmul_rn(__fmul_rn(1.f - a.b2, g), g));
+    const float p = __fsub_rn(master, __fdiv_rn(__fmul_rn(m, a.step_size), __fadd_rn(sqrtf(v), a.eps)));
+    master = __fmul_rn(__fmaf_rn(1.f - a.decay, p, __fmul_rn(__fmul_rn(a.decay, master), a.debias_old)), a.debias_new);
+    return master;
+}
diff --git a/jnerf_b200/lib.py b/jnerf_b200/lib.py
--- a/jnerf_b200/lib.py
+++ b/jnerf_b200/lib.py
@@ -23,6 +23,8 @@
     "ngp_mlp_param_count": (_i32, [_u32]),
     "ngp_network_fwd": (_i32, [_vp, _u32, _vp, _vp, _vp, _vp, _vp, _vp, _vp, _vp]),
     "ngp_network_bwd": (_i32, [_vp, _u32, _vp, _vp, _vp, _vp, _vp, _vp, _vp, _vp, _vp, _vp]),
+    "ngp_network_bwd_fx_bytes": (_i32, [_u64, _vp, _vp]),
+    "ngp_network_bwd_fx": (_i32, [_vp, _u32, _vp, _vp, _vp, _vp, _vp, _vp, _vp, _u32, _vp, _u64, _vp, _u64]),
     "ngp_density_fwd": (_i32, [_vp, _u32, _vp, _vp, _vp, _vp, _vp]),
     "ngp_mesh_workspace_bytes": (_i32, [_u32, _u64, _u64, _vp]),
     "ngp_density_lattice": (_i32, [_vp, _u32, _vp, _vp, _vp, _vp]),
@@ -46,6 +48,9 @@
     "ngp_grid_ema": (_i32, [_vp, _u32, _f32, _vp, _vp]),
     "ngp_grid_update_bitfield": (_i32, [_vp, _vp, _vp, _vp, _u32]),
     "ngp_adam_ema": (_i32, [_vp, _u64, _vp, _i32, _vp, _i32, _f32, _vp, _vp, _vp, _f32, _f32, _f32, _f32, _u32, _f32, _i32]),
+    "ngp_train_sweep": (_i32, [_vp, _u64, _vp, _vp, _vp, _vp, _vp, _vp, _u32, _vp, _vp, _vp, _vp, _vp, _vp, _vp, _vp, _f32, _f32, _f32, _f32, _u32,
+                               _f32]),
+    "ngp_train_sweep_dev": (_i32, [_vp, _u64, _vp, _vp, _vp, _vp, _vp, _vp, _u32, _vp, _vp, _vp, _vp, _vp, _vp, _vp, _vp, _vp]),
     "ngp_dp_exchange_step": (_i32, [_vp, _i32, _i32, _u64, _u32, _vp, _vp, _vp, _vp, _u32, _vp, _vp, _vp, _vp, _vp, _vp, _vp, _f32, _f32, _f32,
                                     _f32, _f32, _u32, _f32]),
     "ngp_dp_exchange_wait": (_i32, [_vp, _i32, _vp, _u32]),
@@ -67,7 +72,7 @@
 
 KERNELS_PER_CALL = {
     "ngp_hash_level_table": 1, "ngp_hash_level_table_primes": 1, "ngp_hash_fwd": 1, "ngp_hash_bwd": 1, "ngp_sh_fwd": 1, "ngp_mlp_fwd": 1, "ngp_mlp_bwd": 1, "ngp_mlp_bwd_dgrad": 1,
-    "ngp_network_fwd": 1, "ngp_network_bwd": 1, "ngp_density_fwd": 1, "ngp_march": 3, "ngp_compact": 1, "ngp_composite_fwd": 1,
+    "ngp_network_fwd": 1, "ngp_network_bwd": 1, "ngp_network_bwd_fx": 1, "ngp_train_sweep": 1, "ngp_train_sweep_dev": 1, "ngp_density_fwd": 1, "ngp_march": 3, "ngp_compact": 1, "ngp_composite_fwd": 1,
     "ngp_composite_bwd": 1, "ngp_composite_infer": 1, "ngp_composite_loss_bwd": 1, "ngp_grid_mark_untrained": 1,
     "ngp_grid_generate_samples": 1, "ngp_grid_splat": 1, "ngp_grid_ema": 1, "ngp_grid_update_bitfield": 7, "ngp_adam_ema": 1, "ngp_dp_exchange_step": 1, "ngp_dp_exchange_wait": 1, "ngp_raygen": 1, "ngp_prepare_batch": 1,
     "ngp_blend_target": 1, "ngp_step_state_set": 1, "ngp_step_state_tick": 1, "ngp_prepare_batch_dev": 1, "ngp_march_dev": 3, "ngp_adam_ema_dev": 1,
diff --git a/jnerf_b200/ops.py b/jnerf_b200/ops.py
--- a/jnerf_b200/ops.py
+++ b/jnerf_b200/ops.py
@@ -106,6 +106,35 @@
 def network_bwd(coords, enc, levels, wd, wr, dout, grid_grad, dwd, dwr, n_dev=None):
     lib.call("ngp_network_bwd", _stream(), coords.shape[0], _p(n_dev), _p(coords), _p(enc), _p(levels.table), _p(wd), _p(wr), _p(dout),
              _p(grid_grad), _p(dwd), _p(dwr))
+
+
+_network_bwd = network_bwd
+
+
+def network_bwd_scratch(levels, device="cuda"):
+    b = np.zeros(2, np.uint64)
+    lib.call("ngp_network_bwd_fx_bytes", levels.n_entries, b.ctypes.data, b[1:].ctypes.data)
+    return (torch.zeros(int(b[0]) // 8, dtype=torch.int64, device=device), torch.zeros(int(b[1]) // 4, dtype=torch.float32, device=device))
+
+
+def network_bwd_fx(coords, enc, levels, wd, wr, dout, fx, w_part, n_dev=None):
+    lib.call("ngp_network_bwd_fx", _stream(), coords.shape[0], _p(n_dev), _p(coords), _p(enc), _p(levels.table), _p(wd), _p(wr), _p(dout),
+             levels.n_entries, _p(fx), fx.numel() * fx.element_size(), _p(w_part), w_part.numel() * w_part.element_size())
+
+
+def _sweep_args(table, table_state, fx, w_part, bwd_rows, wd, wd_state, wr, wr_state):
+    assert table.dtype == wd.dtype == wr.dtype == torch.float16 and table.numel() % 2 == 0
+    return (_stream(), table.numel() // 2, _p(table), *map(_p, table_state), _p(fx), _p(w_part), int(bwd_rows), _p(wd), *map(_p, wd_state), _p(wr),
+            *map(_p, wr_state))
+
+
+def train_sweep(table, table_state, fx, w_part, bwd_rows, wd, wd_state, wr, wr_state, lr, step, beta1=0.9, beta2=0.99, eps=1e-15, ema_decay=0.95):
+    lib.call("ngp_train_sweep", *_sweep_args(table, table_state, fx, w_part, bwd_rows, wd, wd_state, wr, wr_state), float(lr), float(beta1),
+             float(beta2), float(eps), int(step), float(ema_decay))
+
+
+def train_sweep_dev(table, table_state, fx, w_part, bwd_rows, wd, wd_state, wr, wr_state, state):
+    lib.call("ngp_train_sweep_dev", *_sweep_args(table, table_state, fx, w_part, bwd_rows, wd, wd_state, wr, wr_state), _p(state))
 
 
 def density_fwd(pos, grid, levels, wd):
diff --git a/jnerf_b200/runner.py b/jnerf_b200/runner.py
--- a/jnerf_b200/runner.py
+++ b/jnerf_b200/runner.py
@@ -66,6 +66,9 @@
         self.dnet = torch.zeros((cap, 4), dtype=torch.float16, device=dev)
         self.last_loss = None
         self.last_rgb = None
+        self._fx = self._w_part = None
+        if self.world_size == 1 and ops.network_bwd is ops._network_bwd:
+            self._fx, self._w_part = ops.network_bwd_scratch(m.pos_encoder.levels, device=dev)
         if self.world_size == 1:
             self._dev_state = ops.step_state_new()
             self._dev_expect = None
@@ -197,9 +200,12 @@
         rgb, loss, _ = ops.composite_loss_bwd(self.net_out, coords, s._rays_numsteps, s._rays_numsteps_compacted, bg, target,
                                               s.density_grid_mean, delta=self.loss_func.delta, cascades=s.NERF_CASCADES, dnet=self.dnet)
         self.net_backward(coords, n_dev)
-        for p, g in ((m.pos_encoder.m_grid, self.grid_grad), (m.density_mlp.con_weights, self.dwd), (m.rgb_mlp.con_weights, self.dwr)):
-            stp = self._st[id(p)]
-            ops.adam_ema_dev(p.data, g, stp.m, stp.v, stp.master, st, zero_grad=True)
+        if self._fx is not None:
+            ops.train_sweep_dev(*self._sweep_tensors(), st)
+        else:
+            for p, g in ((m.pos_encoder.m_grid, self.grid_grad), (m.density_mlp.con_weights, self.dwd), (m.rgb_mlp.con_weights, self.dwr)):
+                stp = self._st[id(p)]
+                ops.adam_ema_dev(p.data, g, stp.m, stp.v, stp.master, st, zero_grad=True)
         ops.step_state_tick(st, R, lr_next, adam.betas[0], adam.betas[1], adam.eps, self.ema_optimizer.decay, 1.0)
         self.last_loss, self.last_rgb = loss, rgb
         return loss
@@ -366,7 +372,7 @@
         self.ema_optimizer.steps += 1
         m = self.model
         hyper = (lr, adam.n_step, adam.betas[0], adam.betas[1], adam.eps, self.ema_optimizer.decay)
-        if self.world_size > 1:
+        if self.world_size > 1 or self._fx is not None:
             self._optimizer_step(lr, adam.n_step)
             return self._pipe_finish(F, loss, rgb, batch, next_batch)
         P["bwd_done"].record(main)
@@ -489,13 +495,27 @@
 
     def net_backward(self, coords, n_dev):
         m = self.model
+        if self._fx is not None:
+            ops.network_bwd_fx(coords, self.enc, m.pos_encoder.levels, m.density_mlp.con_weights, m.rgb_mlp.con_weights, self.dnet,
+                               self._fx, self._w_part, n_dev=n_dev)
+            self._bwd_rows = coords.shape[0]
+            return
         ops.network_bwd(coords, self.enc, m.pos_encoder.levels, m.density_mlp.con_weights, m.rgb_mlp.con_weights, self.dnet,
                         self.grid_grad, self.dwd, self.dwr, n_dev=n_dev)
+
+    def _sweep_tensors(self):
+        m = self.model
+        st = [self._st[id(p)] for p in (m.pos_encoder.m_grid, m.density_mlp.con_weights, m.rgb_mlp.con_weights)]
+        return (m.pos_encoder.m_grid.data, (st[0].m, st[0].v, st[0].master), self._fx, self._w_part, self._bwd_rows,
+                m.density_mlp.con_weights.data, (st[1].m, st[1].v, st[1].master), m.rgb_mlp.con_weights.data, (st[2].m, st[2].v, st[2].master))
 
     def _optimizer_step(self, lr, n_step):
         m = self.model
         adam = self.optimizer._nested_optimizer
         hyper = (lr, n_step, adam.betas[0], adam.betas[1], adam.eps, self.ema_optimizer.decay)
+        if self._fx is not None:
+            ops.train_sweep(*self._sweep_tensors(), lr, n_step, adam.betas[0], adam.betas[1], adam.eps, self.ema_optimizer.decay)
+            return
         if self.world_size > 1 and self.dp_mode == "p2p":
             st = self._st[id(m.pos_encoder.m_grid)]
             self._epoch += 1
```

After: 3.322 million (median of 6 runs). 7.9% higher.
